# jirsat/wavenets

Hardware: NVIDIA B200
Metric: audio samples/sec fwd+bwd WaveNet stack (higher is better)
Workload: dtype bf16

## Files before the change

### wavenets_b200/csrc/gemm_tc_stack_bwd.cuh

```cuda
#pragma once
#include "gemm_tc_stack.cuh"

#ifdef TC_TIMELINE
#define SBT_DECL(n) long long sbt[n] = {}; long long sbt_prev = clock64();
#define SBT(i) { const long long sbt_now = clock64(); sbt[i] += sbt_now - sbt_prev; sbt_prev = sbt_now; }
#else
#define SBT_DECL(n)
#define SBT(i)
#endif

struct alignas(128) TcStackBwdLayer {
  CUtensorMap tmDX, tmDS, tmWdg, tmZf, tmZs, tmDZ, tmWb, tmDXp, tmO;
  int shift[TC_MAX_TAPS];
  int has_dx, has_ds, has_res;
  int wait_dx;
  const uint8_t* mask;
  int kind, out_mode, act, kb_tap, in_flag_layer;
  int alias;
};

struct TcStackBwdParams {
  int B, T, tiles_t, num_mtiles, L;
  int nseg;
  int kb_dx, kb_ds;
  unsigned long long pol_dx, pol_ds, pol_w, pol_z, pol_dz_ld, pol_dz_st, pol_o;
  float drop_scale;
  int relaxed_handoff;
  int band, nbands;
};

template <int D_, int R_, bool V2 = false> struct TcStackBwdCfg {
  static constexpr int BM = 128, BK = 64;
  static constexpr int A_BYTES = BM * BK * 2;
  static constexpr int B_BYTES = 128 * BK * 2;
  static constexpr int STAGE_BYTES = A_BYTES + B_BYTES;
  static constexpr int STAGES = V2 ? 5 : 3;
  static constexpr int NSLAB = 2 * D_ / 64;
  static constexpr int NPAIR = D_ / 64;
  static constexpr int DZ_SLOTS = V2 ? 0 : 4;
  static constexpr int DZ_BYTES = DZ_SLOTS * A_BYTES;
  static constexpr int PANEL = 128 * 64;
  static constexpr int IN_SLOTS = 3, OUT_SLOTS = 2;
  static constexpr int TMEM_COLS = 512;
  static constexpr int SMEM_BYTES = STAGES * STAGE_BYTES + DZ_BYTES + IN_SLOTS * 2 * PANEL + OUT_SLOTS * PANEL + 512;
  static_assert(D_ % 128 == 0 && D_ <= 256 && R_ % 64 == 0 && R_ <= 256, "stack backward kernel: D in {128,256}, R <= 256");
  static_assert(SMEM_BYTES <= 232448, "stack backward kernel does not fit shared memory");
};

template <int D_, int R_, bool V2>
__global__ void __launch_bounds__(416, 1)
tc_stack_bwd_kernel(const TcStackBwdLayer* __restrict__ layers, int* __restrict__ flags_dx, int* __restrict__ flags_dz, const TcStackBwdParams p) {
  using Cfg = TcStackBwdCfg<D_, R_, V2>;
  constexpr int STAGES = Cfg::STAGES, NEPI = 8, NPAIR = Cfg::NPAIR;
  constexpr int KB_Z = Cfg::NSLAB;
  extern __shared__ __align__(1024) uint8_t smem_sb[];
  uint8_t* smem = smem_sb;
  if ((smem_u32(smem) & 1023u) != 0u) { if (threadIdx.x == 0) printf("libwavenet_b200: dynamic shared memory is not 1024-byte aligned\n"); __trap(); }
  uint8_t* dzbuf = smem + STAGES * Cfg::STAGE_BYTES;
  uint8_t* in_ring = dzbuf + Cfg::DZ_BYTES;
  uint8_t* out_ring = in_ring + Cfg::IN_SLOTS * 2 * Cfg::PANEL;
  uint64_t* full_bar = (uint64_t*)(out_ring + Cfg::OUT_SLOTS * Cfg::PANEL);
  uint64_t* empty_bar = full_bar + STAGES;
  uint64_t* dg_full = empty_bar + STAGES;
  uint64_t* dg_empty = dg_full + 1;
  uint64_t* out_full = dg_empty + 1;
  uint64_t* out_empty = out_full + 1;
  uint64_t* in_full = out_empty + 1;
  uint64_t* in_empty = in_full + Cfg::IN_SLOTS;
  uint64_t* oslot_empty = in_empty + Cfg::IN_SLOTS;
  uint64_t* slab_done = oslot_empty + Cfg::OUT_SLOTS;
  uint64_t* slab_full = slab_done + 2;
  uint64_t* slab_cons = slab_full + 2;
  uint64_t* slab_free = slab_cons + 2;
  uint64_t* a_done = slab_free + 2;
  uint64_t* a_ready = a_done + STAGES;
  uint64_t* sfree = a_ready + STAGES;
  uint32_t* tmem_ptr = (uint32_t*)(sfree + STAGES);
  auto tile_ksteps = [&](const TcStackBwdLayer& Ly, int& n_dg, int& n_un, int& n_sh) {
    if (Ly.kind) { n_dg = 0; n_un = 0; n_sh = p.nseg * Ly.kb_tap; }
    else { n_dg = (Ly.has_dx ? p.kb_dx : 0) + (Ly.has_ds ? p.kb_ds : 0); n_un = KB_Z; n_sh = (p.nseg - 1) * KB_Z; }
  };
  auto ring_adv = [&](int& rs, uint32_t& rp, int n) { rs += n; while (rs >= STAGES) { rs -= STAGES; rp ^= 1u; } };

  const int warp = threadIdx.x >> 5, lane = threadIdx.x & 31;
  const uint32_t crank = cluster_ctarank();
  const bool leader = crank == 0;
  const int tile_first = (int)blockIdx.x >> 1, tile_stride = (int)gridDim.x >> 1;
  const int pair_row0 = (int)crank * Cfg::BM;
  const int total_tiles = p.L * p.num_mtiles;
  const int n_tiles = tile_first < total_tiles ? (total_tiles - tile_first + tile_stride - 1) / tile_stride : 0;

  auto locate = [&](int j, int& ly, int& mt, int& b, int& tb) {
    const int gt = tile_first + j * tile_stride;
    const int full = (p.nbands - 1) * p.band * p.L;
    int lr, mr;
    if (gt < full) {
      const int k = gt / (p.band * p.L), r = gt - k * (p.band * p.L);
      lr = r / p.band; mr = k * p.band + (r - lr * p.band);
    } else {
      const int wl = p.num_mtiles - (p.nbands - 1) * p.band, r = gt - full;
      lr = r / wl; mr = (p.nbands - 1) * p.band + (r - lr * wl);
    }
    ly = p.L - 1 - lr;
    b = mr / p.tiles_t;
    tb = p.tiles_t - 1 - (mr - b * p.tiles_t);
    mt = b * p.tiles_t + tb;
  };

  if (warp == 1 && lane == 0) {
    for (int i = 0; i < STAGES; ++i) { mbar_init(&full_bar[i], 1); mbar_init(&empty_bar[i], 1); }
    mbar_init(dg_full, 1); mbar_init(dg_empty, NEPI * 2); mbar_init(out_full, 1); mbar_init(out_empty, NEPI * 2);
    for (int i = 0; i < Cfg::IN_SLOTS; ++i) { mbar_init(&in_full[i], 1); mbar_init(&in_empty[i], NEPI); }
    for (int i = 0; i < Cfg::OUT_SLOTS; ++i) mbar_init(&oslot_empty[i], 1);
    for (int i = 0; i < 2; ++i) { mbar_init(&slab_done[i], NEPI); mbar_init(&slab_full[i], 2); mbar_init(&slab_cons[i], 1); mbar_init(&slab_free[i], 1); }
    for (int i = 0; i < STAGES; ++i) { mbar_init(&a_done[i], NEPI); mbar_init(&a_ready[i], 2); mbar_init(&sfree[i], 1); }
    mbar_fence_init();
  }
  if (warp == 2) tmem_alloc_pair<Cfg::TMEM_COLS>(tmem_ptr);
  tc_fence_before();
  __syncthreads();
  cluster_sync_all();
  tc_fence_after();
  const uint32_t tmem_base = *tmem_ptr;
  pdl_launch_dependents();
  pdl_wait();

  auto wait_flag = [&](const int* f, int ly, int mt) {
    const long long spin0 = clock64();
    while (ld_acquire_gpu(f) < 2) {
      __nanosleep(32);
      if (clock64() - spin0 > 6000000000ll) { printf("libwavenet_b200: stack backward waited > 3 s for tile (%d, %d)\n", ly, mt); __trap(); }
    }
  };

  if (warp == 0) {
    if (lane == 0) {
      int stage = 0; uint32_t phase = 0;
      auto next = [&]() { if (++stage == STAGES) { stage = 0; phase ^= 1; } };
      uint32_t un_pend = 0u, un_wpar = 0u, un_npar = 0u;
      auto stage_wait = [&]() {
        mbar_wait(&empty_bar[stage], phase ^ 1);
        if (V2 && ((un_pend >> stage) & 1u)) { mbar_wait(&sfree[stage], (un_wpar >> stage) & 1u); un_pend &= ~(1u << stage); }
      };
      SBT_DECL(4)
      constexpr int WDG_BYTES = (D_ / 2) * 64 * 2, WB_BYTES = (R_ / 2) * 64 * 2;
      for (int j = 0; j < n_tiles; ++j) {
        int ly, mt, b, tb;
        locate(j, ly, mt, b, tb);
        const TcStackBwdLayer& Ly = layers[ly];
        const int t0 = tb * (2 * Cfg::BM) + pair_row0;
        if (Ly.kind) {
          for (int s = 0; s < p.nseg; ++s) {
            const int lo = tb * (2 * Cfg::BM) + Ly.shift[s];
            const int t_lo = lo / (2 * Cfg::BM);
            int t_hi = (lo + 2 * Cfg::BM - 1) / (2 * Cfg::BM);
            if (t_hi > p.tiles_t - 1) t_hi = p.tiles_t - 1;
            SBT(0)
            for (int tt = t_lo; tt <= t_hi; ++tt) wait_flag(flags_dx + (size_t)(ly + 1) * p.num_mtiles + b * p.tiles_t + tt, ly + 1, b * p.tiles_t + tt);
            SBT(1)
          }
          fence_proxy_async_global();
          for (int s = 0; s < p.nseg; ++s)
            for (int kb = 0; kb < Ly.kb_tap; ++kb) {
              stage_wait();
              uint8_t* sa = smem + stage * Cfg::STAGE_BYTES;
              if (leader) mbar_expect_tx(&full_bar[stage], 2 * (Cfg::A_BYTES + WB_BYTES));
              tma_load_3d_pair_h(sa, &Ly.tmDZ, &full_bar[stage], kb * 64, t0 + Ly.shift[s], b, p.pol_dz_ld);
              tma_load_2d_pair_h(sa + Cfg::A_BYTES, &Ly.tmWb, &full_bar[stage], (s * Ly.kb_tap + kb) * 64, (int)crank * (R_ / 2), p.pol_w);
              next();
            }
          continue;
        }
        if (Ly.has_dx) {
          if (Ly.wait_dx) {
            SBT(0)
            wait_flag(flags_dx + (size_t)(ly + 1) * p.num_mtiles + mt, ly + 1, mt);
            fence_proxy_async_global();
            SBT(1)
          }
          for (int kb = 0; kb < p.kb_dx; ++kb) {
            stage_wait();
            uint8_t* sa = smem + stage * Cfg::STAGE_BYTES;
            if (leader) mbar_expect_tx(&full_bar[stage], 2 * (Cfg::A_BYTES + WDG_BYTES));
            tma_load_4d_pair_h(sa, &Ly.tmDX, &full_bar[stage], kb * 64, t0, b, 0, p.pol_dx);
            tma_load_2d_pair_h(sa + Cfg::A_BYTES, &Ly.tmWdg, &full_bar[stage], kb * 64, (int)crank * (D_ / 2), p.pol_w);
            next();
          }
        }
        if (Ly.has_ds) {
          const int k0 = (Ly.has_dx && !Ly.alias) ? p.kb_dx * 64 : 0;
          for (int kb = 0; kb < p.kb_ds; ++kb) {
            stage_wait();
            uint8_t* sa = smem + stage * Cfg::STAGE_BYTES;
            if (leader) mbar_expect_tx(&full_bar[stage], 2 * (Cfg::A_BYTES + WDG_BYTES));
            tma_load_4d_pair_h(sa, &Ly.tmDS, &full_bar[stage], kb * 64, t0, b, 0, p.pol_ds);
            tma_load_2d_pair_h(sa + Cfg::A_BYTES, &Ly.tmWdg, &full_bar[stage], k0 + kb * 64, (int)crank * (D_ / 2), p.pol_w);
            next();
          }
        }
        const int kloc = (p.nseg - 1) * 2 * D_;
        for (int pr = 0; pr < NPAIR; ++pr) {
          for (int hh = 0; hh < 2; ++hh) {
            const int slab = hh == 0 ? pr : NPAIR + pr;
            stage_wait();
            uint8_t* sa = smem + stage * Cfg::STAGE_BYTES;
            if (leader) mbar_expect_tx(&full_bar[stage], 2 * WB_BYTES);
            tma_load_2d_pair_h(sa + Cfg::A_BYTES, &Ly.tmWb, &full_bar[stage], kloc + slab * 64, (int)crank * (R_ / 2), p.pol_w);
            if (V2) {
              un_wpar = (un_wpar & ~(1u << stage)) | (((un_npar >> stage) & 1u) << stage);
              un_npar ^= 1u << stage; un_pend |= 1u << stage;
            }
            next();
          }
        }
        for (int s = 0; s < p.nseg - 1; ++s) {
          const int lo = tb * (2 * Cfg::BM) + Ly.shift[s];
          const int t_lo = lo / (2 * Cfg::BM);
          int t_hi = (lo + 2 * Cfg::BM - 1) / (2 * Cfg::BM);
          if (t_hi > p.tiles_t - 1) t_hi = p.tiles_t - 1;
          SBT(0)
          for (int tt = t_lo; tt <= t_hi; ++tt) wait_flag(flags_dz + (size_t)ly * p.num_mtiles + b * p.tiles_t + tt, ly, b * p.tiles_t + tt);
          fence_proxy_async_global();
          SBT(2)
          for (int kb = 0; kb < KB_Z; ++kb) {
            stage_wait();
            uint8_t* sa = smem + stage * Cfg::STAGE_BYTES;
            if (leader) mbar_expect_tx(&full_bar[stage], 2 * (Cfg::A_BYTES + WB_BYTES));
            tma_load_3d_pair_h(sa, &Ly.tmDZ, &full_bar[stage], kb * 64, t0 + Ly.shift[s], b, p.pol_dz_ld);
            tma_load_2d_pair_h(sa + Cfg::A_BYTES, &Ly.tmWb, &full_bar[stage], s * 2 * D_ + kb * 64, (int)crank * (R_ / 2), p.pol_w);
            next();
          }
        }
      }
      SBT(0)
#ifdef TC_TIMELINE
      if (blockIdx.x == 0 || blockIdx.x == 41)
        printf("SBWD cta %d producer: tiles %d  ring+issue %lld  wait_flag_dx %lld  wait_flag_dz %lld\n", blockIdx.x, n_tiles, sbt[0], sbt[1], sbt[2]);
#endif
    }
  } else if (warp == 1) {
    if (leader) {
      constexpr uint32_t idesc_g = umma_idesc_bf16(256, D_, 0, 0);
      constexpr uint32_t idesc_o = umma_idesc_bf16(256, R_, 0, 0);
      const uint32_t t_dg = tmem_base, t_out = tmem_base + 256u;
      int stage = 0; uint32_t phase = 0;
      uint32_t n_sf[2] = {0u, 0u};
      uint32_t ng = 0u;
      uint32_t ar_par = 0u;
      SBT_DECL(10)
      auto kstep = [&](uint32_t d_tmem, uint32_t idesc, bool a_from_dz, int slot, bool first, uint64_t* extra0, uint64_t* extra1) {
#ifdef TC_TIMELINE
        const long long w0 = clock64();
#endif
        mbar_wait(&full_bar[stage], phase);
#ifdef TC_TIMELINE
        sbt[9] += clock64() - w0;
#endif
        tc_fence_after();
        if (elect_one()) {
          const uint32_t sa = smem_u32(smem + stage * Cfg::STAGE_BYTES);
          const uint32_t a_addr = a_from_dz ? smem_u32(dzbuf) + (uint32_t)slot * (uint32_t)Cfg::A_BYTES : sa;
          const uint64_t adesc = umma_smem_desc(a_addr, 16, 1024);
          const uint64_t bdesc = umma_smem_desc(sa + Cfg::A_BYTES, 16, 1024);
#pragma unroll
          for (int k = 0; k < Cfg::BK / 16; ++k)
            umma_bf16_pair(d_tmem, adesc + (uint64_t)(2 * k), bdesc + (uint64_t)(2 * k), idesc, (first && k == 0) ? 0u : 1u);
          umma_commit_pair(&empty_bar[stage]);
          if (extra0) umma_commit_pair(extra0);
          if (extra1) umma_commit_pair(extra1);
        }
        __syncwarp();
        if (++stage == STAGES) { stage = 0; phase ^= 1; }
      };
      for (int j = 0; j < n_tiles; ++j) {
        int ly, mt, b, tb;
        locate(j, ly, mt, b, tb);
        const TcStackBwdLayer& Ly = layers[ly];
        const uint32_t par = (uint32_t)(j & 1);
        if (Ly.kind) {
          SBT(2)
          mbar_wait(out_empty, par ^ 1);
          SBT(3)
          tc_fence_after();
          const int ks_p = p.nseg * Ly.kb_tap;
          for (int ks = 0; ks < ks_p; ++ks) kstep(t_out, idesc_o, false, 0, ks == 0, ks == ks_p - 1 ? out_full : nullptr, nullptr);
          SBT(7)
          continue;
        }
        const uint32_t gpar = ng & 1u; ++ng;
        SBT(0)
        mbar_wait(dg_empty, gpar ^ 1);
        SBT(1)
        tc_fence_after();
        const int ks_dg = (Ly.has_dx ? p.kb_dx : 0) + (Ly.has_ds ? p.kb_ds : 0);
        for (int ks = 0; ks < ks_dg; ++ks) kstep(t_dg, idesc_g, false, 0, ks == 0, ks == ks_dg - 1 ? dg_full : nullptr, nullptr);
        SBT(2)
        mbar_wait(out_empty, par ^ 1);
        SBT(3)
        tc_fence_after();
        const int ks_sh = (p.nseg - 1) * KB_Z;
        bool first = true;
        if constexpr (V2) {
          for (int q = 0; q < KB_Z; ++q) {
            if ((q & 1) == 0) { mbar_wait(&a_ready[stage], (ar_par >> stage) & 1u); ar_par ^= 1u << stage; }
            SBT(5)
            tc_fence_after();
            const bool last = ks_sh == 0 && q == KB_Z - 1;
            kstep(t_out, idesc_o, false, 0, first, last ? out_full : nullptr, nullptr); first = false;
            SBT(6)
          }
        } else
        for (int pr = 0; pr < NPAIR; ++pr) {
          const int ps = pr & 1;
          mbar_wait(&slab_full[ps], n_sf[ps] & 1u); ++n_sf[ps];
          SBT(5)
          tc_fence_after();
          const bool last = ks_sh == 0 && pr == NPAIR - 1;
          kstep(t_out, idesc_o, true, 2 * ps, first, nullptr, nullptr); first = false;
          kstep(t_out, idesc_o, true, 2 * ps + 1, false, &slab_cons[ps], last ? out_full : nullptr);
          SBT(6)
        }
        for (int ks = 0; ks < ks_sh; ++ks) kstep(t_out, idesc_o, false, 0, false, ks == ks_sh - 1 ? out_full : nullptr, nullptr);
        SBT(7)
      }
#ifdef TC_TIMELINE
      if (lane == 0 && (blockIdx.x == 0 || blockIdx.x == 40))
        printf("SBWD cta %d mma: tiles %d  wait_dg_empty %lld  DG ksteps %lld  wait_out_empty %lld  wait_slab_full %lld  unshifted %lld  shifted %lld  (of the ksteps: wait_full_bar %lld)\n",
               blockIdx.x, n_tiles, sbt[1], sbt[2], sbt[3], sbt[5], sbt[6], sbt[7], sbt[9]);
#endif
    }
  } else if (warp == 2) {
    int oslot = 0;
    uint64_t* pend = nullptr;
    uint64_t* pend2 = nullptr;
    auto committed = [&](uint64_t* rel, uint64_t* rel2 = nullptr) {
      bulk_commit_group();
      if (pend) { bulk_wait_group_read<1>(); mbar_arrive(pend); if (pend2) mbar_arrive(pend2); }
      pend = rel; pend2 = rel2;
    };
    int s_rs = 0; uint32_t s_rp = 0u;
    auto publish = [&](int* flag) {
      bulk_wait_group<0>();
      if (pend) { mbar_arrive(pend); if (pend2) mbar_arrive(pend2); pend = nullptr; pend2 = nullptr; }
      fence_proxy_async_global();
      __threadfence();
      red_release_gpu_add(flag, 1);
    };
    for (int j = 0; j < n_tiles; ++j) {
      int ly, mt, b, tb;
      locate(j, ly, mt, b, tb);
      const TcStackBwdLayer& Ly = layers[ly];
      const int t0 = tb * (2 * Cfg::BM) + pair_row0;
      int n_dg, n_un, n_sh;
      tile_ksteps(Ly, n_dg, n_un, n_sh);
      if (!Ly.kind) {
      int u_rs = s_rs; uint32_t u_rp = s_rp;
      ring_adv(u_rs, u_rp, n_dg);
      for (int pr = 0; pr < NPAIR; ++pr) {
        const int ps = pr & 1;
        if constexpr (V2) {
          named_bar_sync(8 + pr, NEPI * 32 + 32);
          const int sf = u_rs; ring_adv(u_rs, u_rp, 1);
          const int ss = u_rs; ring_adv(u_rs, u_rp, 1);
          if (lane == 0) {
            tma_store_3d_h(smem + sf * Cfg::STAGE_BYTES, &Ly.tmDZ, pr * 64, t0, b, p.pol_dz_st);
            tma_store_3d_h(smem + ss * Cfg::STAGE_BYTES, &Ly.tmDZ, D_ + pr * 64, t0, b, p.pol_dz_st);
            committed(&sfree[sf], &sfree[ss]);
          }
        } else {
        named_bar_sync(8 + ps, NEPI * 32 + 32);
        if (lane == 0) {
          tma_store_3d_h(dzbuf + (2 * ps) * Cfg::A_BYTES, &Ly.tmDZ, pr * 64, t0, b, p.pol_dz_st);
          tma_store_3d_h(dzbuf + (2 * ps + 1) * Cfg::A_BYTES, &Ly.tmDZ, D_ + pr * 64, t0, b, p.pol_dz_st);
          committed(&slab_free[ps]);
        }
        }
        __syncwarp();
      }
      if (lane == 0) publish(flags_dz + (size_t)ly * p.num_mtiles + mt);
      __syncwarp();
      }
      for (int step = 0; step < R_ / 32; ++step) {
        named_bar_sync(3 + oslot, NEPI * 32 + 32);
        if (lane == 0) {
          tma_store_3d_h(out_ring + oslot * Cfg::PANEL, &Ly.tmO, step * 32, t0, b, p.pol_o);
          committed(&oslot_empty[oslot]);
        }
        __syncwarp();
        if (++oslot == Cfg::OUT_SLOTS) oslot = 0;
      }
      if (lane == 0) publish(flags_dx + (size_t)ly * p.num_mtiles + mt);
      __syncwarp();
      ring_adv(s_rs, s_rp, n_dg + n_un + n_sh);
    }
    if (lane == 0) bulk_wait_group<0>();
  } else if (warp == 3) {
    if (lane == 0) {
      int islot = 0; uint32_t iphase = 0;
      for (int j = 0; j < n_tiles; ++j) {
        int ly, mt, b, tb;
        locate(j, ly, mt, b, tb);
        const TcStackBwdLayer& Ly = layers[ly];
        const int t0 = tb * (2 * Cfg::BM) + pair_row0;
        if (!Ly.kind)
        for (int step = 0; step < D_ / 32; ++step) {
          mbar_wait(&in_empty[islot], iphase ^ 1);
          mbar_expect_tx(&in_full[islot], 2u * Cfg::PANEL);
          uint8_t* dst = in_ring + islot * 2 * Cfg::PANEL;
          tma_load_3d_h(dst, &Ly.tmZf, &in_full[islot], step * 32, t0, b, p.pol_z);
          tma_load_3d_h(dst + Cfg::PANEL, &Ly.tmZs, &in_full[islot], step * 32, t0, b, p.pol_z);
          if (++islot == Cfg::IN_SLOTS) { islot = 0; iphase ^= 1; }
        }
        if (Ly.out_mode) {
          if (Ly.in_flag_layer >= 0) {
            wait_flag(flags_dx + (size_t)Ly.in_flag_layer * p.num_mtiles + mt, Ly.in_flag_layer, mt);
            fence_proxy_async_global();
          }
          for (int step = 0; step < R_ / 32; ++step) {
            mbar_wait(&in_empty[islot], iphase ^ 1);
            mbar_expect_tx(&in_full[islot], (uint32_t)Cfg::PANEL);
            tma_load_3d_h(in_ring + islot * 2 * Cfg::PANEL, &Ly.tmDXp, &in_full[islot], step * 32, t0, b, p.pol_dx);
            if (++islot == Cfg::IN_SLOTS) { islot = 0; iphase ^= 1; }
          }
        }
      }
    }
  } else if (warp == 12) {
    if (lane == 0) {
      uint32_t n_sd[2] = {0u, 0u};
      int h_rs = 0; uint32_t h_rp = 0u, ad_par = 0u;
      for (int j = 0; j < n_tiles; ++j) {
        int n_dg, n_un, n_sh;
        { int ly, mt, b, tb; locate(j, ly, mt, b, tb); tile_ksteps(layers[ly], n_dg, n_un, n_sh); }
        if constexpr (V2) {
          int u_rs = h_rs; uint32_t u_rp = h_rp;
          ring_adv(u_rs, u_rp, n_dg);
          for (int q = 0; q < n_un; q += 2) {
            mbar_wait(&a_done[u_rs], (ad_par >> u_rs) & 1u); ad_par ^= 1u << u_rs;
            if (leader) mbar_arrive(&a_ready[u_rs]);
            else if (p.relaxed_handoff) mbar_arrive_remote_relaxed(&a_ready[u_rs], 0u);
            else mbar_arrive_remote(&a_ready[u_rs], 0u);
            ring_adv(u_rs, u_rp, 2);
          }
          ring_adv(h_rs, h_rp, n_dg + n_un + n_sh);
          continue;
        }
        if (n_un == 0) continue;
        for (int pr = 0; pr < NPAIR; ++pr) {
          const int ps = pr & 1;
          mbar_wait(&slab_done[ps], n_sd[ps] & 1u); ++n_sd[ps];
          if (leader) mbar_arrive(&slab_full[ps]);
          else if (p.relaxed_handoff) mbar_arrive_remote_relaxed(&slab_full[ps], 0u);
          else mbar_arrive_remote(&slab_full[ps], 0u);
        }
      }
    }
  } else if (warp >= 4 && warp < 12) {
    const int e = warp - 4;
    const int quarter = warp & 3;
    const int q = e >> 2;
    const int row = quarter * 32 + lane;
    const uint32_t row_off = (uint32_t)row * 64u;
    const uint32_t sw = (uint32_t)((row >> 1) & 3);
    const uint32_t u0 = (uint32_t)(2 * q), u1 = u0 + 1;
    const uint32_t off0 = row_off + ((u0 ^ sw) << 4), off1 = row_off + ((u1 ^ sw) << 4);
    const uint32_t grow = (uint32_t)row * 128u, gsw = (uint32_t)(row & 7);
    int islot = 0; uint32_t iphase = 0;
    int oslot = 0; uint32_t ophase = 0;
    uint32_t n_use[2] = {0u, 0u};
    uint32_t nge = 0u;
    int e_rs = 0; uint32_t e_rp = 0u;
    uint32_t eu_pend = 0u, eu_wpar = 0u, eu_npar = 0u;
    uint8_t* slab_dst[2] = {nullptr, nullptr};
    int slab_st[2] = {0, 0};
    const TcEpiGateBwd<true>::Params pg{D_};
    const uint32_t lane_base = (uint32_t)(quarter * 32) << 16;
    SBT_DECL(10)
    for (int j = 0; j < n_tiles; ++j) {
      const uint32_t par = (uint32_t)(j & 1);
      int out_mode, out_act, kind;
      int n_dg, n_un, n_sh;
      const uint8_t* mrow = nullptr;
      {
        int ly, mt, b, tb;
        locate(j, ly, mt, b, tb);
        out_mode = layers[ly].out_mode; out_act = layers[ly].act; kind = layers[ly].kind;
        tile_ksteps(layers[ly], n_dg, n_un, n_sh);
        const int tt = tb * (2 * Cfg::BM) + pair_row0 + row;
        if (layers[ly].mask && tt < p.T && b < p.B) mrow = layers[ly].mask + ((size_t)b * p.T + tt) * R_;
      }
      if (!kind) {
      const uint32_t gpar = nge & 1u; ++nge;
      SBT(0)
      mbar_wait(dg_full, gpar);
      SBT(1)
      tc_fence_after();
      int u_rs = e_rs; uint32_t u_rp = e_rp;
      ring_adv(u_rs, u_rp, n_dg);
      {
        TmemAccRow acc{tmem_base + lane_base, true};
#pragma unroll 1
        for (int step = 0; step < D_ / 32; ++step) {
          const int pr = step >> 1, ps = pr & 1;
          float in[2][16];
          float out[2][16];
          SBT(2)
          mbar_wait(&in_full[islot], iphase);
          SBT(3)
          {
            const uint8_t* ib = in_ring + islot * 2 * Cfg::PANEL;
#pragma unroll
            for (int k = 0; k < 2; ++k) {
              const uint4 a = *reinterpret_cast<const uint4*>(ib + k * Cfg::PANEL + off0);
              const uint4 c = *reinterpret_cast<const uint4*>(ib + k * Cfg::PANEL + off1);
              const uint32_t w[8] = {a.x, a.y, a.z, a.w, c.x, c.y, c.z, c.w};
#pragma unroll
              for (int i = 0; i < 8; ++i) {
                in[k][2 * i] = __uint_as_float(w[i] << 16);
                in[k][2 * i + 1] = __uint_as_float(w[i] & 0xffff0000u);
              }
            }
          }
          __syncwarp();
          if (lane == 0) mbar_arrive(&in_empty[islot]);
          if (++islot == Cfg::IN_SLOTS) { islot = 0; iphase ^= 1; }
          TcEpiGateBwd<true>::chunk(pg, acc, 0, step * 32 + q * 16, 0, 0, 3u, in, out, nullptr);
          SBT(2)
          if constexpr (V2) {
            if ((step & 1) == 0) {
#pragma unroll
              for (int k = 0; k < 2; ++k) {
                mbar_wait(&empty_bar[u_rs], u_rp ^ 1u);
                if ((eu_pend >> u_rs) & 1u) { mbar_wait(&sfree[u_rs], (eu_wpar >> u_rs) & 1u); eu_pend &= ~(1u << u_rs); }
                eu_wpar = (eu_wpar & ~(1u << u_rs)) | (((eu_npar >> u_rs) & 1u) << u_rs);
                eu_npar ^= 1u << u_rs; eu_pend |= 1u << u_rs;
                slab_st[k] = u_rs; slab_dst[k] = smem + u_rs * Cfg::STAGE_BYTES;
                ring_adv(u_rs, u_rp, 1);
              }
            }
          } else
          if ((step & 1) == 0 && n_use[ps] > 0) {
            mbar_wait(&slab_cons[ps], (n_use[ps] - 1u) & 1u);
            mbar_wait(&slab_free[ps], (n_use[ps] - 1u) & 1u);
          }
          SBT(4)
          {
            const int ch = (step & 1) * 32 + q * 16;
            const uint32_t j0 = (uint32_t)(ch >> 3);
#pragma unroll
            for (int k = 0; k < 2; ++k) {
              uint8_t* gs = (V2 ? slab_dst[k] : dzbuf + (2 * ps + k) * Cfg::A_BYTES) + grow;
              uint4 a, c;
              a.x = pack_bf16x2(out[k][0], out[k][1]); a.y = pack_bf16x2(out[k][2], out[k][3]);
              a.z = pack_bf16x2(out[k][4], out[k][5]); a.w = pack_bf16x2(out[k][6], out[k][7]);
              c.x = pack_bf16x2(out[k][8], out[k][9]); c.y = pack_bf16x2(out[k][10], out[k][11]);
              c.z = pack_bf16x2(out[k][12], out[k][13]); c.w = pack_bf16x2(out[k][14], out[k][15]);
              *reinterpret_cast<uint4*>(gs + ((j0 ^ gsw) << 4)) = a;
              *reinterpret_cast<uint4*>(gs + (((j0 + 1) ^ gsw) << 4)) = c;
            }
          }
          if (step & 1) {
            fence_proxy_async();
            named_bar_arrive(8 + (V2 ? pr : ps), NEPI * 32 + 32);
            __syncwarp();
            if constexpr (V2) {
              if (lane == 0) mbar_arrive(&a_done[slab_st[0]]);
            } else {
              if (lane == 0) mbar_arrive(&slab_done[ps]);
            }
            ++n_use[ps];
          }
        }
      }
      tc_fence_before();
      __syncwarp();
      if (lane == 0) mbar_arrive_remote_relaxed(dg_empty, 0u);
      }
      SBT(2)
      mbar_wait(out_full, par);
      SBT(5)
      tc_fence_after();
      {
        TmemAccRow acc{tmem_base + 256u + lane_base, true};
#pragma unroll 1
        for (int step = 0; step < R_ / 32; ++step) {
          float v[16];
          acc.load16(step * 32 + q * 16, v);
          if (mrow) {
            const uint4 mk = __ldg(reinterpret_cast<const uint4*>(mrow + step * 32 + q * 16));
            const uint32_t mw[4] = {mk.x, mk.y, mk.z, mk.w};
#pragma unroll
            for (int i = 0; i < 16; ++i) v[i] = ((mw[i >> 2] >> (8 * (i & 3))) & 0xffu) ? v[i] * p.drop_scale : 0.f;
          }
          if (out_mode) {
            mbar_wait(&in_full[islot], iphase);
            const uint8_t* ib = in_ring + islot * 2 * Cfg::PANEL;
            const uint4 a = *reinterpret_cast<const uint4*>(ib + off0);
            const uint4 c = *reinterpret_cast<const uint4*>(ib + off1);
            const uint32_t w[8] = {a.x, a.y, a.z, a.w, c.x, c.y, c.z, c.w};
            float y[16];
#pragma unroll
            for (int i = 0; i < 8; ++i) {
              y[2 * i] = __uint_as_float(w[i] << 16);
              y[2 * i + 1] = __uint_as_float(w[i] & 0xffff0000u);
            }
            if (out_mode == 1) {
#pragma unroll
              for (int i = 0; i < 16; ++i) v[i] += y[i];
            } else {
              wn_act_grad16(out_act, y, v);
            }
            __syncwarp();
            if (lane == 0) mbar_arrive(&in_empty[islot]);
            if (++islot == Cfg::IN_SLOTS) { islot = 0; iphase ^= 1; }
          }
          uint8_t* ob = out_ring + oslot * Cfg::PANEL;
          SBT(6)
          mbar_wait(&oslot_empty[oslot], ophase ^ 1);
          SBT(7)
          uint4 a, c;
          a.x = pack_bf16x2(v[0], v[1]); a.y = pack_bf16x2(v[2], v[3]); a.z = pack_bf16x2(v[4], v[5]); a.w = pack_bf16x2(v[6], v[7]);
          c.x = pack_bf16x2(v[8], v[9]); c.y = pack_bf16x2(v[10], v[11]); c.z = pack_bf16x2(v[12], v[13]); c.w = pack_bf16x2(v[14], v[15]);
          *reinterpret_cast<uint4*>(ob + off0) = a;
          *reinterpret_cast<uint4*>(ob + off1) = c;
          fence_proxy_async();
          named_bar_arrive(3 + oslot, NEPI * 32 + 32);
          if (++oslot == Cfg::OUT_SLOTS) { oslot = 0; ophase ^= 1; }
        }
      }
      tc_fence_before();
      __syncwarp();
      if (lane == 0) mbar_arrive_remote_relaxed(out_empty, 0u);
      ring_adv(e_rs, e_rp, n_dg + n_un + n_sh);
      SBT(6)
    }
#ifdef TC_TIMELINE
    if (lane == 0 && warp == 4 && (blockIdx.x == 0 || blockIdx.x == 41))
      printf("SBWD cta %d epilogue warp 4: wait_dg_full %lld  DG epi work %lld (+ wait z panels %lld, wait slab slot %lld)  wait_out_full %lld  OUT epi work %lld (+ wait out slot %lld)\n",
             blockIdx.x, sbt[1], sbt[2], sbt[3], sbt[4], sbt[5], sbt[6], sbt[7]);
#endif
  }
  tc_fence_before();
  __syncthreads();
  cluster_sync_all();
  if (warp == 2) tmem_dealloc_pair<Cfg::TMEM_COLS>(tmem_base);
}

struct TcStackBwdDesc {
  int B, T, nseg, shift[TC_MAX_TAPS], D, R, S;
  const bf16* dxo;
  const bf16* dskip; int lds;
  const bf16* z;
  bf16* dz;
  bf16* dx;
  const bf16* Wdg; int k_dg;
  const bf16* Wb; int k_b;
  int has_res;
  const uint8_t* mask; float drop_scale;
  int plain; const bf16* gin;
  int out_mode, act, ein_layer; const bf16* ein;
  int alias;
};

struct TcStackBwdPlan {
  int B = 0, T = 0, L = 0, num_mtiles = 0; bool drop = false;
  TcStackBwdLayer* d_layers = nullptr; int* d_flags = nullptr;
  void release() { cudaFree(d_layers); cudaFree(d_flags); d_layers = nullptr; d_flags = nullptr; }
};

template <int D_, int R_>
static int tc_stack_bwd_build_t(TmapCache& tc, const std::vector<TcStackBwdDesc>& descs, TcStackBwdPlan* plan) {
  std::vector<TcStackBwdLayer> tab(descs.size());
  for (size_t l = 0; l < descs.size(); ++l) {
    const TcStackBwdDesc& d = descs[l];
    TcStackBwdLayer& t = tab[l];
    memset(&t, 0, sizeof(t));
    const TcEpiIo xo{d.dx, d.R, d.R, 0};
    const CUtensorMap* mO = tc_panel_map(tc, xo, d.T, d.B);
    uint64_t bd[2] = {(uint64_t)d.k_b, (uint64_t)d.R}, bs[1] = {(uint64_t)d.k_b * 2};
    uint32_t bb[2] = {64, (uint32_t)(R_ / 2)};
    const CUtensorMap* mWb = tc.get(d.Wb, 2, bd, bs, bb);
    if (!mO || !mWb) return -10;
    t.tmO = *mO; t.tmWb = *mWb; t.tmDXp = *mO;
    for (int s = 0; s < TC_MAX_TAPS; ++s) t.shift[s] = s < d.nseg ? d.shift[s] : 0;
    t.mask = d.mask;
    t.kind = d.plain ? 1 : 0; t.out_mode = d.out_mode; t.act = d.act; t.in_flag_layer = d.out_mode == 1 ? d.ein_layer : -1;
    if (d.out_mode) {
      const TcEpiIo ei{d.ein, d.R, d.R, 0};
      const CUtensorMap* mp = tc_panel_map(tc, ei, d.T, d.B);
      if (!mp) return -10;
      t.tmDXp = *mp;
    }
    if (d.plain) {
      const CUtensorMap* mG = tc_slab_map(tc, d.gin, d.D, d.D, d.T, d.B);
      if (!mG) return -10;
      t.tmDZ = *mG; t.kb_tap = d.D / 64;
      t.tmDX = *mG; t.tmDS = *mG; t.tmWdg = *mWb; t.tmZf = *mO; t.tmZs = *mO;
      continue;
    }
    const CUtensorMap* mDZ = tc_slab_map(tc, d.dz, 2 * d.D, 2 * d.D, d.T, d.B);
    const TcEpiIo zf{d.z, 2 * d.D, d.D, 0}, zs{d.z + d.D, 2 * d.D, d.D, 0};
    const CUtensorMap* mZf = tc_panel_map(tc, zf, d.T, d.B);
    const CUtensorMap* mZs = tc_panel_map(tc, zs, d.T, d.B);
    uint64_t wd[2] = {(uint64_t)d.k_dg, (uint64_t)d.D}, ws[1] = {(uint64_t)d.k_dg * 2};
    uint32_t wb[2] = {64, (uint32_t)(D_ / 2)};
    const CUtensorMap* mWdg = tc.get(d.Wdg, 2, wd, ws, wb);
    if (!mDZ || !mZf || !mZs || !mWdg) return -10;
    t.tmDZ = *mDZ; t.tmZf = *mZf; t.tmZs = *mZs; t.tmWdg = *mWdg;
    t.tmDX = *mDZ; t.tmDS = *mDZ;
    if (d.dxo) {
      const CUtensorMap* m = tc_act_map(tc, d.dxo, d.R, d.R, d.T, d.B, 1, 0, 128);
      if (!m) return -10;
      t.tmDX = *m;
    }
    if (d.dskip) {
      const CUtensorMap* m = tc_act_map(tc, d.dskip, d.lds, d.S, d.T, d.B, 1, 0, 128);
      if (!m) return -10;
      t.tmDS = *m;
    }
    t.has_dx = d.dxo != nullptr; t.has_ds = d.dskip != nullptr; t.has_res = d.out_mode == 1 ? 1 : 0; t.alias = d.alias;
    t.wait_dx = (d.dxo != nullptr && l + 1 < descs.size()) ? 1 : 0;
  }
  const TcStackBwdDesc& d0 = descs[0];
  plan->release();
  plan->B = d0.B; plan->T = d0.T; plan->L = (int)descs.size(); plan->num_mtiles = d0.B * ((d0.T + 255) / 256); plan->drop = false;
  for (const TcStackBwdDesc& d : descs) if (d.mask) plan->drop = true;
  if (cudaMalloc((void**)&plan->d_layers, tab.size() * sizeof(TcStackBwdLayer)) != cudaSuccess ||
      cudaMemcpy(plan->d_layers, tab.data(), tab.size() * sizeof(TcStackBwdLayer), cudaMemcpyHostToDevice) != cudaSuccess ||
      cudaMalloc((void**)&plan->d_flags, (size_t)2 * plan->L * plan->num_mtiles * sizeof(int)) != cudaSuccess) {
    snprintf(g_tc_err, sizeof(g_tc_err), "stack backward: plan allocation failed: %s", cudaGetErrorString(cudaGetLastError()));
    plan->release();
    return -23;
  }
  return 0;
}

template <int D_, int R_, bool V2>
static int tc_stack_bwd_launch_t(cudaStream_t st, const TcStackBwdPlan& plan, const TcStackBwdDesc& d0) {
  using Cfg = TcStackBwdCfg<D_, R_, V2>;
  TcStackBwdParams p{};
  p.B = d0.B; p.T = d0.T; p.tiles_t = (d0.T + 255) / 256; p.num_mtiles = d0.B * p.tiles_t; p.L = plan.L;
  p.nseg = d0.nseg; p.kb_dx = d0.R / 64; p.kb_ds = d0.S / 64; p.drop_scale = d0.drop_scale;
  p.pol_dx = tc_policy(TC_L2_NORMAL); p.pol_ds = tc_policy(TC_L2_LAST); p.pol_w = tc_policy(TC_L2_LAST); p.pol_z = tc_policy(TC_L2_FIRST);
  p.pol_dz_ld = tc_policy(TC_L2_NORMAL); p.pol_dz_st = tc_policy(TC_L2_LAST); p.pol_o = tc_policy(TC_L2_LAST);
  auto kern = tc_stack_bwd_kernel<D_, R_, V2>;
  static unsigned long long attr_devs = 0ull;
  if (tc_first_use_on_device(&attr_devs)) {
    cudaError_t e = cudaFuncSetAttribute(kern, cudaFuncAttributeMaxDynamicSharedMemorySize, Cfg::SMEM_BYTES);
    if (e != cudaSuccess) { snprintf(g_tc_err, sizeof(g_tc_err), "cudaFuncSetAttribute(smem=%d): %s", Cfg::SMEM_BYTES, cudaGetErrorString(e)); return -12; }
  }
  const int pairs = tc_num_sms() / 2;
  if (p.num_mtiles <= pairs) return -100;
  {
    static int relaxed = -1;
    if (relaxed < 0) { const char* e = getenv("WN_TC_HANDOFF_RELAXED"); relaxed = (e && e[0] == '1') ? 1 : 0; }
    p.relaxed_handoff = relaxed;
    static int band_target = -1;
    if (band_target < 0) { const char* e = getenv("WN_TC_SB_BAND"); band_target = e ? atoi(e) : 128; }
    int nb = band_target > 0 ? p.num_mtiles / band_target : 1;
    if (nb < 1) nb = 1;
    for (; nb > 1; --nb) {
      const int bw = (p.num_mtiles + nb - 1) / nb;
      if (bw > pairs && p.num_mtiles - (nb - 1) * bw > pairs) break;
    }
    p.nbands = nb; p.band = (p.num_mtiles + nb - 1) / nb;
  }
  {
    static int max_clusters_dev[64];
    static unsigned long long mc_devs = 0ull;
    int& max_clusters = max_clusters_dev[tc_current_device()];
    if (tc_first_use_on_device(&mc_devs)) {
      cudaLaunchConfig_t oc{};
      oc.gridDim = dim3(tc_num_sms()); oc.blockDim = dim3(416); oc.dynamicSmemBytes = Cfg::SMEM_BYTES;
      cudaLaunchAttribute oa[1];
      oa[0].id = cudaLaunchAttributeClusterDimension;
      oa[0].val.clusterDim.x = 2; oa[0].val.clusterDim.y = 1; oa[0].val.clusterDim.z = 1;
      oc.attrs = oa; oc.numAttrs = 1;
      int n = 0;
      if (cudaOccupancyMaxActiveClusters(&n, kern, &oc) != cudaSuccess) { n = 0; cudaGetLastError(); }
      max_clusters = n;
    }
    if (pairs > max_clusters) return -100;
  }
  const size_t nflags = (size_t)plan.L * plan.num_mtiles;
  if (cudaMemsetAsync(plan.d_flags, 0, 2 * nflags * sizeof(int), st) != cudaSuccess) return -14;
  cudaLaunchConfig_t cfg{};
  cfg.gridDim = dim3(2 * pairs); cfg.blockDim = dim3(416); cfg.dynamicSmemBytes = Cfg::SMEM_BYTES; cfg.stream = st;
  cudaLaunchAttribute attr[2];
  cfg.attrs = attr; cfg.numAttrs = tc_launch_attrs(attr, 2);
  cudaError_t e = cudaLaunchKernelEx(&cfg, kern, (const TcStackBwdLayer*)plan.d_layers, plan.d_flags, plan.d_flags + nflags, p);
  if (e != cudaSuccess) { snprintf(g_tc_err, sizeof(g_tc_err), "stack backward launch: %s", cudaGetErrorString(e)); return -13; }
  return 0;
}

static inline int tc_stack_bwd_build(TmapCache& tc, const std::vector<TcStackBwdDesc>& descs, TcStackBwdPlan* plan) {
  const TcStackBwdDesc& d = descs[0];
  if (d.D == 256 && d.R == 256) return tc_stack_bwd_build_t<256, 256>(tc, descs, plan);
  if (d.D == 128 && d.R == 128) return tc_stack_bwd_build_t<128, 128>(tc, descs, plan);
  return -100;
}
static inline int tc_stack_bwd_launch(cudaStream_t st, const TcStackBwdPlan& plan, const TcStackBwdDesc& d, bool v2) {
  if (d.D == 256 && d.R == 256) return v2 ? tc_stack_bwd_launch_t<256, 256, true>(st, plan, d) : tc_stack_bwd_launch_t<256, 256, false>(st, plan, d);
  if (d.D == 128 && d.R == 128) return v2 ? tc_stack_bwd_launch_t<128, 128, true>(st, plan, d) : tc_stack_bwd_launch_t<128, 128, false>(st, plan, d);
  return -100;
}
```

### wavenets_b200/csrc/wn_api.cu

```cuda
#include <cuda_runtime.h>
#include <math.h>
#include <stdarg.h>
#include <stdio.h>
#include <stdlib.h>
#include <string.h>

#include <algorithm>
#include <string>
#include <vector>

#include "../../include/wavenet_b200.h"
#include "common.cuh"
#include "epilogues.cuh"
#include "gemm_simt.cuh"
#include "gemm_tc.cuh"
#include "gemm_tc_block.cuh"
#include "gemm_tc_wgroup.cuh"
#include "gemm_tc_stack.cuh"
#include "gemm_tc_stack_bwd.cuh"
#include "kernels_misc.cuh"
#include "generate.cuh"
#include "nccl_dl.cuh"

static thread_local char g_err[512] = "";
static void set_err(const char* fmt, ...) {
  va_list ap;
  va_start(ap, fmt);
  vsnprintf(g_err, sizeof(g_err), fmt, ap);
  va_end(ap);
}
extern "C" const char* wn_last_error(void) { return g_err; }
extern "C" const char* wn_build_info(void) {
  return "libwavenet_b200 sm_100a; fp32 FFMA tier + bf16 tcgen05/TMEM/TMA tier; built " __DATE__ " " __TIME__;
}

#define CK(expr)                                                                          \
  do {                                                                                    \
    cudaError_t e_ = (expr);                                                              \
    if (e_ != cudaSuccess) {                                                              \
      set_err("CUDA error %s (%s) at %s:%d", cudaGetErrorName(e_), cudaGetErrorString(e_), __FILE__, __LINE__); \
      return WN_ERR_CUDA;                                                                 \
    }                                                                                     \
  } while (0)
#define RET(expr)              \
  do {                         \
    int r_ = (expr);           \
    if (r_ != WN_OK) return r_; \
  } while (0)

static inline int cdiv(long long a, long long b) { return (int)((a + b - 1) / b); }
static inline int rup(int a, int b) { return (a + b - 1) / b * b; }

struct ParamInfo {
  std::string name;
  int shape[3];
  int ndim;
  long long offset, count;
};

struct ConvP {
  int K = 1, cin = 0, cout = 0, dil = 1;
  int w_idx = -1, b_idx = -1;
  bool gate = false;
  float* Wf = nullptr; int Npad = 0;
  float* Wb = nullptr; int Cpad = 0;
  bf16* Wf16 = nullptr; int Kf16 = 0;
  bf16* Wb16 = nullptr; int Kb16 = 0;
  int N16 = 0, C16 = 0, tileN16 = 0;
};

struct BlockP {
  std::vector<ConvP> stack;
  ConvP conv1;
  bool has_skip = false;
  ConvP conv_skip;
  bool has_cond = false;
  int cw_idx = -1, cb_idx = -1;
  float* Wdg = nullptr; int Dpad = 0;
  bf16* Wdg16 = nullptr;
  bf16* Wres16 = nullptr;
  float* Wfc = nullptr;
  float* Wct = nullptr; int Ccpad = 0;
  bf16* Wfc16 = nullptr; int Kfc16 = 0;
  bf16* Wct16 = nullptr; int Cc16 = 0, tileCc16 = 0;
};

struct Arena {
  char* base = nullptr;
  size_t cap = 0, off = 0;
  bool dry = true;
  void* take(size_t bytes) {
    off = (off + 255) & ~(size_t)255;
    void* p = dry ? nullptr : base + off;
    off += bytes;
    return p;
  }
};

struct wn_handle {
  wn_config cfg;
  int R, D, S, Sp , K, L, Cc, Cout;
  bool alias_skip;
  std::vector<int> dil;
  int rf;
  std::vector<ParamInfo> params;
  long long n_scalars = 0;
  float* d_params = nullptr;
  float* d_grads = nullptr;
  ConvP input_conv;
  std::vector<BlockP> blocks;
  std::vector<ConvP> head;
  std::vector<int> map_w, map_b, map_width;
  float* Wskip = nullptr; int Spad = 0;
  bf16* Wskip16 = nullptr;
  float* bskip_sum = nullptr;
  int* d_bskip_offsets = nullptr;
  int* d_cond_offsets = nullptr;
  Arena pack, ws;
  int maxB, maxT;
  void* h0 = nullptr;
  std::vector<std::vector<void*>> acts;
  std::vector<void*> zbuf, xout;
  void* G_all = nullptr;
  void* skipsum = nullptr;
  std::vector<void*> hact;
  float* logits = nullptr; int ldl = 0;
  void* dlogits = nullptr; int ldd = 0;
  void *dhA = nullptr, *dhB = nullptr;
  void* dskip = nullptr;
  void *dxA = nullptr, *dxB = nullptr, *dotmp = nullptr;
  void *dcatA = nullptr, *dcatB = nullptr;
  void* dz = nullptr;
  void *dpA = nullptr, *dpB = nullptr;
  float* colpart = nullptr; int col_chunks = 0;
  float* wg_partial = nullptr; long long wg_partial_elems = 0;
  float* cs_partial = nullptr;
  float* wg_partial_side = nullptr; float* cs_partial_side = nullptr;
  void* dz2 = nullptr;
  float* loss_partial = nullptr; int loss_parts_cap = 0;
  float* cond_act[WN_MAX_LIST + 1] = {};
  float* cond_dact = nullptr;
  float* cond_dact2 = nullptr;
  float* cb = nullptr;
  float* dcb = nullptr;
  float* dcond = nullptr;
  float* l2_sum = nullptr;
  uint8_t* drop_mask = nullptr;
  std::vector<void*> xdrop;
  void* ddrop = nullptr;
  unsigned long long* d_drop_ctr = nullptr;
  unsigned long long drop_seed = 0x243F6A8885A308D3ull;
  bool drop_injected = false;
  bool drop_active = false;
  float* opt_m = nullptr; float* opt_v = nullptr;
  OptChunk* opt_chunks = nullptr; int opt_n_chunks = 0;
  int* opt_var_first = nullptr;
  float* opt_partial = nullptr; float* opt_scale = nullptr; float* opt_norms = nullptr;
  float opt_lr = 1e-3f, opt_b1 = 0.9f, opt_b2 = 0.999f, opt_eps = 1e-7f, opt_clipnorm = 0.f;
  long long opt_t = 0;
  float* layer_xin = nullptr;
  void* layer_in = nullptr;
  float* d_loss = nullptr;
  float* d_frames = nullptr; float* d_cond_in = nullptr;
  float* pin_frames = nullptr; float* pin_cond = nullptr; float* pin_loss = nullptr;
  cudaStream_t own_stream = nullptr;
  int lastB = 0, lastT = 0;
  bool fwd_valid = false;
  bool layer_fwd_valid[WN_MAX_DILATIONS] = {};
  bool layer_drop[WN_MAX_DILATIONS] = {};
  int Ccs = 0;
  std::vector<void*> cseq;
  float* cseq_bias = nullptr;
  float* cseq_dw = nullptr;
  const void* layer_cseq[WN_MAX_DILATIONS] = {};
  const void* cond_seq = nullptr;
  const float* last_cond = nullptr;
  long long launches = 0;
  int prof_tag = 0;
  std::vector<std::pair<cudaEvent_t, cudaEvent_t>> prof_events;
  std::vector<const char*> prof_labels;
  const char* cur_label = "misc";
  const char* outer_label = nullptr;
  std::vector<float> prof_ms;
  std::vector<const char*> prof_last_labels;
  size_t prof_used = 0;
  long long prof_launches = 0;
  TmapCache tmaps;
  struct StepGraph { const float* frames; const float* cond; int B, T, nrep; float* loss; bool train; int seen; long long launches; cudaGraphExec_t exec; };
  std::vector<StepGraph> graphs;
  int use_graphs = 1;
  cudaEvent_t ev_in = nullptr, ev_out = nullptr;
  cudaStream_t side_stream = nullptr;
  std::vector<cudaEvent_t> ev_blk_in, ev_blk_dz, ev_blk_done;
  int use_side = 1;
  int use_res_gemm = 1;
  int use_fused_fwd = 1;
  int stack_fwd_layers = 0;
  int use_stack_fwd = 1;
  std::vector<TcStackPlan> stack_plans;
  int use_stack_bwd = 2, stack_bwd_layers = 0;
  std::vector<TcStackBwdPlan> stack_bwd_plans;
  int tile_gate_bwd = 0, tile_dgrad = 0;
  int fused_fwd_launches = 0;
  int use_group_wgrad = 0;
  void* dz_all = nullptr;
  void* dx_all = nullptr;
  void* do_all = nullptr;
  std::vector<std::vector<void*>> dp_keep;
  struct WgPlan { int B, T; bool drop; bool sb; int nb; TcWgGroupPlan plan; };
  std::vector<WgPlan> wg_plans;
  std::vector<TcWgJobDesc> wg_jobs;
  int dskip_l2_last = 0;
  int wg_last_tiles = 0, wg_last_side = 0;
  int wg_last_partials = 0;
  int wg_cur_group = -1;
  int wg_side_every = 5;
  cudaEvent_t ev_wg_side = nullptr;
  int wg_force_split = 0, wg_pair_tiles = 1;
  int use_merged_finish = 0;
  struct Gen {
    int B = 0, cap = 0;
    float* audio = nullptr; std::vector<std::vector<float*>> hist; float* z = nullptr; float* skipsum = nullptr;
    std::vector<float*> hbuf; float* logits = nullptr; float* sampled = nullptr; int* t_dev = nullptr;
    std::vector<float*> wcat, bcat;
    std::vector<void*> allocs;
  } gen;
  TcWgradFinish pend_finish{}; bool pend_valid = false; int pend_blocks = 0; long long pend_partial_elems = 0, pend_cs_elems = 0;
  std::vector<PackJob> pack_jobs;
  PackJob* d_pack_jobs = nullptr; long long pack_blocks = 0; bool pack_ready = false;
  wn_ncclComm_t comm = nullptr; bool comm_owned = false; int comm_nranks = 1, comm_rank = 0;
  int ar_in_step = 0;
  int ar_buckets = 2;
  int ar_first_pct = 70;
  bool ar_now = false;
  long long ar_early_lo = -1, ar_early_hi = -1;
  cudaStream_t comm_stream = nullptr;
  cudaEvent_t ev_bucket[8] = {nullptr, nullptr, nullptr, nullptr, nullptr, nullptr, nullptr, nullptr};
  cudaEvent_t ev_comm_done = nullptr;
  int wg_cur_bucket = 0;
  int last_ar_buckets = 0;
  bool cond_wgrad_done = false;
};

enum { CLS_DILATED = 1, CLS_GEMM = 2, CLS_LOSS = 3, CLS_MISC = 4 };

struct LaunchScope {
  wn_handle* h; cudaStream_t st; bool timed = false; size_t slot = 0;
  LaunchScope(wn_handle* h_, cudaStream_t st_, int cls) : h(h_), st(st_) {
    h->launches++;
    const int t = h->prof_tag;
    if (t && ((t == 1 && cls == CLS_DILATED) || (t == 2 && (cls == CLS_DILATED || cls == CLS_GEMM)) || (t == 3 && cls == CLS_LOSS) ||
              (t == 4))) {
      if (h->prof_used == h->prof_events.size()) {
        cudaEvent_t a, b;
        cudaEventCreate(&a); cudaEventCreate(&b);
        h->prof_events.push_back({a, b});
      }
      slot = h->prof_used++;
      if (h->prof_labels.size() <= slot) h->prof_labels.resize(slot + 1);
      h->prof_labels[slot] = h->outer_label ? h->outer_label : h->cur_label;
      cudaEventRecord(h->prof_events[slot].first, st);
      timed = true;
      h->prof_launches++;
    }
  }
  ~LaunchScope() {
    if (timed) cudaEventRecord(h->prof_events[slot].second, st);
  }
};

struct OuterLabel {
  wn_handle* h; const char* prev;
  OuterLabel(wn_handle* h_, const char* l) : h(h_), prev(h_->outer_label) { h->outer_label = l; }
  ~OuterLabel() { h->outer_label = prev; }
};

static int add_param(wn_handle* h, const std::string& name, std::initializer_list<int> shape) {
  ParamInfo p;
  p.name = name;
  p.ndim = (int)shape.size();
  p.count = 1;
  int i = 0;
  for (int s : shape) { p.shape[i++] = s; p.count *= s; }
  for (; i < 3; ++i) p.shape[i] = 1;
  p.offset = h->n_scalars;
  h->n_scalars += (p.count + 3) / 4 * 4;
  h->params.push_back(p);
  return (int)h->params.size() - 1;
}

static int validate_config(const wn_config& c) {
  if (c.conditioning != 0 && c.conditioning != 1) { set_err("Conditioning must be 'global', 'local' or None."); return c.conditioning == 2 ? WN_ERR_UNSUPPORTED : WN_ERR_VALUE; }
  if (c.kernel_size < 2) { set_err("Kernel size must be at least 2."); return WN_ERR_VALUE; }
  if (c.dilation_bound < 1) { set_err("dilation bound must be power of kernel_size."); return WN_ERR_VALUE; }
  {
    long long v = 1; bool ok = false;
    for (int i = 0; i < 40 && v <= c.dilation_bound; ++i) { if (v == c.dilation_bound) { ok = true; break; } v *= c.kernel_size; }
    if (!ok && c.n_dilations == 0) { set_err("dilation bound must be power of kernel_size."); return WN_ERR_VALUE; }
  }
  if (c.layers_per_block < 1) { set_err("Layers per block must be at least 1."); return WN_ERR_VALUE; }
  if (c.blocks < 1) { set_err("Blocks must be at least 1."); return WN_ERR_VALUE; }
  if (c.num_mixtures < 0) { set_err("Number of mixtures must be at least 1 or None."); return WN_ERR_VALUE; }
  if (c.dropout < 0 || c.dropout > 1) { set_err("Dropout must be between 0 and 1."); return WN_ERR_VALUE; }
  if (c.sampling_function < 0 || c.sampling_function > 2) { set_err("Sampling function must be categorical, logistic or gaussian."); return WN_ERR_VALUE; }
  if (c.sampling_function == WN_CATEGORICAL && c.num_mixtures != 0) { set_err("Categorical sampling cannot be used with mixtures."); return WN_ERR_VALUE; }
  if (c.has_head && c.sampling_function != WN_CATEGORICAL && c.num_mixtures == 0) { set_err("mixture sampling needs num_mixtures"); return WN_ERR_VALUE; }
  if (c.channels < 1 || c.max_batch < 1 || c.max_time < 1) { set_err("channels / max_batch / max_time must be positive"); return WN_ERR_VALUE; }
  if (c.kernel_size > WN_MAX_TAPS) { set_err("kernel_size > %d not built", WN_MAX_TAPS); return WN_ERR_UNSUPPORTED; }
  if (c.num_mixtures > WN_MAX_MIX) { set_err("num_mixtures > %d not built", WN_MAX_MIX); return WN_ERR_UNSUPPORTED; }
  if (c.blocks * c.layers_per_block > WN_MAX_DILATIONS) { set_err("too many dilated convs"); return WN_ERR_UNSUPPORTED; }
  if (c.n_mapping < 0 || c.n_mapping > WN_MAX_LIST || c.n_final < 0 || c.n_final > WN_MAX_LIST) { set_err("list too long"); return WN_ERR_VALUE; }
  if (c.has_head && c.sampling_function == WN_CATEGORICAL && (c.bits < 1 || c.bits > 16)) { set_err("bits must be in 1..16"); return WN_ERR_VALUE; }
  if (c.conditioning && c.cond_in < 1) { set_err("conditioning needs cond_in >= 1"); return WN_ERR_VALUE; }
  if (c.precision != WN_FP32 && c.precision != WN_BF16) { set_err("unknown precision"); return WN_ERR_VALUE; }
  return WN_OK;
}

static ConvP make_conv(wn_handle* h, const std::string& pfx, int K, int cin, int cout, int dil, bool gate) {
  ConvP c;
  c.K = K; c.cin = cin; c.cout = cout; c.dil = dil; c.gate = gate;
  c.w_idx = add_param(h, pfx + "/kernel", {K, cin, cout});
  c.b_idx = add_param(h, pfx + "/bias", {cout});
  return c;
}

template <class T> static size_t esz() { return sizeof(T); }

static void layout_buffers(wn_handle* h) {
  const bool bf = h->cfg.precision == WN_BF16;
  const size_t es = bf ? 2 : 4;
  Arena& P = h->pack;
  auto lay_conv = [&](ConvP& c) {
    if (!bf) {
      c.Npad = rup(c.cout, 64);
      c.Wf = (float*)P.take((size_t)c.K * c.cin * c.Npad * 4);
      c.Cpad = rup(c.cin, 64);
      c.Wb = (float*)P.take((size_t)c.K * c.cout * c.Cpad * 4);
    } else {
      tc_pick_tile(c.cout, c.gate, &c.N16, &c.tileN16);
      c.Kf16 = c.K * c.cin;
      c.Wf16 = (bf16*)P.take((size_t)c.N16 * c.Kf16 * 2);
      int tn;
      tc_pick_tile(c.cin, false, &c.C16, &tn);
      c.Kb16 = c.K * c.cout;
      c.Wb16 = (bf16*)P.take((size_t)c.C16 * rup(c.Kb16, 64) * 2);
    }
  };
  if (h->cfg.has_input_conv) {  }
  for (auto& b : h->blocks) {
    for (auto& c : b.stack) lay_conv(c);
    lay_conv(b.conv1);
    if (b.has_skip) lay_conv(b.conv_skip);
    const int rs = h->R + (b.has_skip ? h->S : 0);
    if (!bf) {
      b.Dpad = rup(h->D, 64);
      b.Wdg = (float*)P.take((size_t)rs * b.Dpad * 4);
    } else {
      int n16, tn;
      tc_pick_tile(h->D, false, &n16, &tn);
      b.Dpad = n16;
      b.Wdg16 = (bf16*)P.take((size_t)n16 * rup(rs, 64) * 2);
      if (h->cfg.use_residual) b.Wres16 = (bf16*)P.take((size_t)b.conv1.N16 * (h->D + h->R) * 2);
    }
    if (b.has_cond && h->Ccs > 0) {
      const ConvP& c = b.stack.back();
      if (!bf) {
        b.Wfc = (float*)P.take((size_t)(c.K * c.cin + h->Cc) * c.Npad * 4);
        b.Ccpad = rup(h->Cc, 64);
        b.Wct = (float*)P.take((size_t)c.cout * b.Ccpad * 4);
      } else {
        b.Kfc16 = c.K * c.cin + h->Ccs;
        b.Wfc16 = (bf16*)P.take((size_t)c.N16 * b.Kfc16 * 2);
        tc_pick_tile(h->Cc, false, &b.Cc16, &b.tileCc16);
        b.Wct16 = (bf16*)P.take((size_t)b.Cc16 * c.cout * 2);
      }
    }
  }
  for (auto& c : h->head) lay_conv(c);
  if (!bf) {
    h->Spad = rup(h->Sp, 64);
    h->Wskip = (float*)P.take((size_t)h->L * h->D * h->Spad * 4);
  } else {
    int tn;
    tc_pick_tile(h->Sp, false, &h->Spad, &tn);
    h->Wskip16 = (bf16*)P.take((size_t)h->Spad * h->L * h->D * 2);
  }
  h->bskip_sum = (float*)P.take((size_t)h->Sp * 4);
  h->d_bskip_offsets = (int*)P.take((size_t)h->L * 4 * 2);
  h->d_cond_offsets = (int*)P.take((size_t)h->L * 4 * 2);

  Arena& W = h->ws;
  const size_t rows = (size_t)h->maxB * h->maxT;
  const int R = h->R, D = h->D, Sp = h->Sp, L = h->L;
  h->h0 = W.take(rows * R * es);
  h->acts.assign(L, {});
  h->zbuf.assign(L, nullptr);
  h->xout.assign(L, nullptr);
  for (int l = 0; l < L; ++l) {
    const int depth = (int)h->blocks[l].stack.size();
    h->acts[l].assign(depth - 1 > 0 ? depth - 1 : 0, nullptr);
    for (int j = 0; j + 1 < depth; ++j) h->acts[l][j] = W.take(rows * D * es);
    h->zbuf[l] = W.take(rows * 2 * D * es);
    h->xout[l] = W.take(rows * R * es);
  }
  h->G_all = W.take((size_t)L * rows * D * es);
  h->skipsum = W.take(rows * Sp * es);
  int maxhead = Sp > R ? Sp : R;
  h->hact.assign(h->head.size() > 0 ? h->head.size() - 1 : 0, nullptr);
  for (size_t i = 0; i + 1 < h->head.size(); ++i) {
    h->hact[i] = W.take(rows * h->head[i].cout * es);
    if (h->head[i].cout > maxhead) maxhead = h->head[i].cout;
  }
  if (h->cfg.has_head) {
    h->ldl = h->Cout;
    h->logits = (float*)W.take(rows * h->ldl * 4);
    h->ldd = bf ? rup(h->Cout, 64) : h->Cout;
    h->dlogits = W.take(rows * h->ldd * es);
    h->dhA = W.take(rows * maxhead * es);
    h->dhB = W.take(rows * maxhead * es);
  }
  h->dskip = W.take(rows * Sp * es);
  h->dxA = W.take(rows * R * es);
  h->dxB = W.take(rows * R * es);
  h->dotmp = W.take(rows * R * es);
  if (h->use_group_wgrad) {
    h->dz_all = W.take((size_t)L * rows * 2 * D * es);
    h->dx_all = W.take((size_t)L * rows * R * es);
    if (h->alias_skip && h->cfg.use_skip) h->do_all = W.take((size_t)L * rows * R * es);
    h->dp_keep.assign(L, {});
    for (int l = 0; l < L; ++l) {
      const int depth = (int)h->blocks[l].stack.size();
      for (int j = 0; j + 1 < depth; ++j) h->dp_keep[l].push_back(W.take(rows * D * es));
    }
  } else if (bf && !h->alias_skip && h->cfg.use_skip) {
    h->dcatA = W.take(rows * (size_t)(R + h->S) * es);
    h->dcatB = W.take(rows * (size_t)(R + h->S) * es);
  }
  h->dz = W.take(rows * 2 * D * es);
  h->dz2 = W.take(rows * 2 * D * es);
  h->dpA = W.take(rows * D * es);
  h->dpB = W.take(rows * D * es);
  h->col_chunks = cdiv(h->maxT, 64);
  int nmax = 2 * D;
  if (R > nmax) nmax = R;
  if (Sp > nmax) nmax = Sp;
  for (auto& c : h->head) if (c.cout > nmax) nmax = c.cout;
  const int kin = (h->K + 1);
  size_t colpart_elems = (size_t)h->maxB * h->col_chunks * (nmax > kin * R ? nmax : kin * R);
  h->colpart = (float*)W.take(colpart_elems * 4);
  long long maxkn = 0;
  auto upd = [&](long long k, long long n) { if ((k + 1) * n > maxkn) maxkn = (k + 1) * n; };
  for (auto& b : h->blocks) {
    for (auto& c : b.stack) upd((long long)c.K * c.cin, c.cout);
    upd(D, R);
    if (b.has_skip) upd(D, h->S);
    if (b.has_cond && h->Ccs > 0) upd(h->Ccs, 2 * D);
  }
  for (auto& c : h->head) upd(c.cin, c.cout);
  h->wg_partial_elems = maxkn * WN_MAX_WGRAD_SPLITS;
  h->wg_partial = (float*)W.take((size_t)h->wg_partial_elems * 4 * 2);
  h->wg_partial_side = (float*)W.take((size_t)h->wg_partial_elems * 4 * 2);
  if (bf) {
    int max_mt = 1;
    auto mt = [&](int K, int cin) { const int m = K * cdiv(cin, 128); if (m > max_mt) max_mt = m; };
    for (auto& b : h->blocks) { for (auto& c : b.stack) mt(c.K, c.cin); mt(1, D); }
    if (h->Ccs > 0) mt(1, h->Ccs);
    for (auto& c : h->head) mt(1, c.cin);
    h->cs_partial = (float*)W.take((size_t)tc_wgrad_cs_rows(h->maxB, h->maxT, max_mt) * (size_t)rup(nmax, 4) * 4 * 2);
    h->cs_partial_side = (float*)W.take((size_t)tc_wgrad_cs_rows(h->maxB, h->maxT, max_mt) * (size_t)rup(nmax, 4) * 4 * 2);
  }
  h->loss_parts_cap = cdiv((long long)rows, 8) + 8;
  h->loss_partial = (float*)W.take((size_t)h->loss_parts_cap * 4);
  int maxw = h->cfg.cond_in;
  for (int i = 0; i < h->cfg.n_mapping; ++i) if (h->cfg.mapping_layers[i] > maxw) maxw = h->cfg.mapping_layers[i];
  if (h->cfg.conditioning) {
    for (int i = 0; i < h->cfg.n_mapping; ++i) h->cond_act[i] = (float*)W.take((size_t)h->maxB * h->cfg.mapping_layers[i] * 4);
    h->cond_dact = (float*)W.take((size_t)h->maxB * maxw * 4);
    h->cond_dact2 = (float*)W.take((size_t)h->maxB * maxw * 4);
    h->cb = (float*)W.take((size_t)L * h->maxB * 2 * D * 4);
    h->dcb = (float*)W.take((size_t)L * h->maxB * 2 * D * 4);
    h->dcond = (float*)W.take((size_t)h->maxB * (h->Cc > 0 ? h->Cc : 1) * 4);
  }
  if (h->Ccs > 0) {
    h->cseq.assign(L, nullptr);
    if (bf) {
      for (int l = 0; l < L; ++l) h->cseq[l] = W.take(rows * h->Ccs * 2);
      h->cseq_dw = (float*)W.take((size_t)h->Ccs * 2 * D * 4);
    }
    h->cseq_bias = (float*)W.take((size_t)L * 2 * D * 4);
  }
  h->l2_sum = (float*)W.take(16);
  if (h->cfg.dropout > 0.f) {
    h->drop_mask = (uint8_t*)W.take((size_t)L * rows * R);
    h->xdrop.assign(L, nullptr);
    for (int l = 0; l < L; ++l) h->xdrop[l] = W.take(rows * R * es);
    h->ddrop = W.take(rows * R * es);
    h->d_drop_ctr = (unsigned long long*)W.take(16);
  }
  h->d_loss = (float*)W.take(16);
  h->layer_in = W.take(rows * R * es);
  h->d_frames = (float*)W.take((size_t)h->maxB * (h->maxT + 1) * 4);
  h->d_cond_in = (float*)W.take((size_t)h->maxB * (h->cfg.cond_in > 0 ? h->cfg.cond_in : 1) * 4);
}
// ... 1088 lines not shown
      for (int k = 0; k < c.K; ++k) g.seg[k] = SegH{dcur, dcw, +(c.K - 1 - k) * c.dil, c.cout};
      fill_w(g, c, true);
      g.tile16 = h->tile_dgrad;
      typename EpiActBwd<T, T>::Params ep{};
      ep.N = c.cin;
      if (j > 0) {
        void* dst = group ? h->dp_keep[l][j - 1] : ((dcur == h->dpA) ? h->dpB : h->dpA);
        ep.out = (T*)dst; ep.ldo = D; ep.add = nullptr; ep.y = (const T*)h->acts[l][j - 1]; ep.ldy = D; ep.act = h->cfg.activation;
        ep.vec = vec_ok<T>(D);
        g.l2_in[1] = TC_L2_FIRST; g.l2_out[0] = TC_L2_LAST;
        RET((run_conv_gemm<T, EpiActBwd<T, T>>(h, st, CLS_DILATED, g, ep)));
        dcur = dst;
        dcw = D;
      } else if (h->drop_active) {
        ep.out = (T*)h->ddrop; ep.ldo = R; ep.add = nullptr; ep.y = nullptr; ep.act = ACT_LINEAR; ep.vec = vec_ok<T>(R);
        RET((run_conv_gemm<T, EpiActBwd<T, T>>(h, st, CLS_DILATED, g, ep)));
        if (sd && sd->wait_dx) CK(cudaStreamWaitEvent(st, sd->wait_dx, 0));
        LaunchScope ls(h, st, CLS_MISC);
        dropout_bwd<T><<<cdiv(nR, 256), 256, 0, st>>>((const T*)h->ddrop, h->drop_mask + (size_t)l * rows_cap * R,
                                                     (h->cfg.use_residual && dxout) ? (const T*)dxout : nullptr, ldxo, (T*)dx_in, ldxi,
                                                     (long long)B * Tn, R, 1.0f / (1.0f - h->cfg.dropout));
      } else {
        ep.out = (T*)dx_in; ep.ldo = ldxi;
        ep.add = (h->cfg.use_residual && dxout) ? (const T*)dxout : nullptr; ep.lda = ldxo;
        ep.y = nullptr; ep.act = ACT_LINEAR; ep.vec = vec_ok<T>(R);
        g.l2_in[0] = TC_L2_FIRST; g.l2_out[0] = TC_L2_LAST;
        if (sd && sd->wait_dx) CK(cudaStreamWaitEvent(st, sd->wait_dx, 0));
        RET((run_conv_gemm<T, EpiActBwd<T, T>>(h, st, CLS_DILATED, g, ep)));
      }
    }
  }
  if (h->pend_valid) {
    LaunchScope ls(h, s1, CLS_GEMM);
    tc_wgrad_finish<<<h->pend_blocks, 256, 0, s1>>>(h->pend_finish);
    h->pend_valid = false;
  }
  if (sd) CK(cudaEventRecord(sd->ev_done, sd->side));
  return WN_OK;
}

static int cond_backward(wn_handle* h, cudaStream_t st, const float* cond_in, const float* cond, int B, int l0, int nl, bool run_mapping, float* dcond_out,
                         float l2coef, bool skip_wgrad = false) {
  const int n = 2 * h->D;
  if (l0 == 0 && nl == h->L) {
    if (!skip_wgrad) {
      LaunchScope ls(h, st, CLS_MISC);
      cond_wgrad_all<<<dim3(cdiv((h->Cc + 1) * n, 128), h->L), 128, 0, st>>>(cond, h->Cc, h->dcb, (long long)h->maxB * n, h->d_params, h->d_grads,
                                                                          h->d_cond_offsets, B, n, l2coef, 0);
    }
    {
      LaunchScope ls(h, st, CLS_MISC);
      cond_dgrad_all<<<B * h->Cc, 256, 0, st>>>(h->dcb, (long long)h->maxB * n, h->d_params, h->d_cond_offsets, dcond_out, h->L, B, h->Cc, n);
    }
  } else
  for (int l = l0; l < l0 + nl; ++l) {
    const BlockP& b = h->blocks[l];
    const float* d = h->dcb + (size_t)l * h->maxB * n;
    {
      LaunchScope ls(h, st, CLS_MISC);
      dense_small_wgrad<<<cdiv((h->Cc + 1) * n, 128), 128, 0, st>>>(cond, h->Cc, d, n, G_(h, b.cw_idx), G_(h, b.cb_idx), B, h->Cc, n);
    }
    if (l2coef != 0.f) {
      LaunchScope ls(h, st, CLS_MISC);
      const long long cnt = h->params[b.cw_idx].count;
      reduce_parts<<<cdiv(cnt, 256), 256, 0, st>>>(G_(h, b.cw_idx), 1, 0, G_(h, b.cw_idx), cnt, P_(h, b.cw_idx), l2coef);
    }
    {
      LaunchScope ls(h, st, CLS_MISC);
      dense_small_dgrad<<<cdiv(B * h->Cc, 4), 128, 0, st>>>(d, n, P_(h, b.cw_idx), dcond_out, h->Cc, B, h->Cc, n, l != l0);
    }
  }
  if (!run_mapping) return WN_OK;
  MapArgs ma;
  if (dcond_out == h->dcond && mapping_args(h, cond_in, B, l2coef, &ma)) {
    LaunchScope ls(h, st, CLS_MISC);
    mapping_bwd_fused<<<1, 256, 0, st>>>(ma);
    return WN_OK;
  }
  float* dcur = dcond_out;
  for (int i = (int)h->map_w.size() - 1; i >= 0; --i) {
    const int nn = h->map_width[i];
    const int kin = i > 0 ? h->map_width[i - 1] : h->cfg.cond_in;
    const float* inp = i > 0 ? h->cond_act[i - 1] : cond_in;
    {
      LaunchScope ls(h, st, CLS_MISC);
      dense_small_actgrad<<<cdiv(B * nn, 128), 128, 0, st>>>(dcur, h->cond_act[i], B * nn, h->cfg.mapping_activation);
    }
    {
      LaunchScope ls(h, st, CLS_MISC);
      dense_small_wgrad<<<cdiv((kin + 1) * nn, 128), 128, 0, st>>>(inp, kin, dcur, nn, G_(h, h->map_w[i]), G_(h, h->map_b[i]), B, kin, nn);
    }
    if (l2coef != 0.f) {
      LaunchScope ls(h, st, CLS_MISC);
      const long long cnt = h->params[h->map_w[i]].count;
      reduce_parts<<<cdiv(cnt, 256), 256, 0, st>>>(G_(h, h->map_w[i]), 1, 0, G_(h, h->map_w[i]), cnt, P_(h, h->map_w[i]), l2coef);
    }
    if (i > 0) {
      float* dn = (dcur == h->cond_dact) ? h->cond_dact2 : h->cond_dact;
      LaunchScope ls(h, st, CLS_MISC);
      dense_small_dgrad<<<cdiv(B * kin, 4), 128, 0, st>>>(dcur, nn, P_(h, h->map_w[i]), dn, kin, B, kin, nn, 0);
      dcur = dn;
    }
  }
  return WN_OK;
}

static const BwdSide* side_setup(wn_handle* h, cudaStream_t st, int l, bool on, BwdSide* sd) {
  if (!on) return nullptr;
  sd->side = h->side_stream;
  sd->ev_in = h->ev_blk_in[l]; sd->ev_dz = h->ev_blk_dz[l]; sd->ev_done = h->ev_blk_done[l];
  sd->wait_dz = l + 2 < h->L ? h->ev_blk_done[l + 2] : nullptr;
  sd->wait_dx = l + 1 < h->L ? h->ev_blk_done[l + 1] : nullptr;
  cudaEventRecord(sd->ev_in, st);
  return sd;
}

template <class T>
static int model_backward(wn_handle* h, cudaStream_t st, const float* x, int ldx, const float* cond_in, int B, int Tn, float l2coef) {
  const wn_config& c = h->cfg;
  const bool group = sizeof(T) == 2 && h->use_group_wgrad;
  const bool use_side = sizeof(T) == 2 && h->use_side && h->prof_tag == 0 && h->side_stream != nullptr && !group;
  const bool cat = sizeof(T) == 2 && h->dcatA != nullptr;
  const int ldc = h->R + h->S;
  const size_t rows_cap = (size_t)h->maxB * h->maxT;
  auto dz_of = [&](int l) -> void* { return (T*)h->dz_all + (size_t)l * rows_cap * 2 * h->D; };
  auto dx_of = [&](int l) -> void* { return (T*)h->dx_all + (size_t)l * rows_cap * h->R; };
  h->wg_jobs.clear();
  h->wg_last_tiles = 0; h->wg_last_side = 0;
  bool sb_ok = false;
  if constexpr (sizeof(T) == 2) {
    sb_ok = group && !cat && h->use_stack_bwd && tc_cta_group() == 2 && h->L >= 2 && h->D == h->R && (h->D == 256 || h->D == 128) &&
            h->K <= TC_MAX_TAPS && B * cdiv(Tn, 256) > tc_num_sms() / 2;
    for (auto& b : h->blocks) {
      if (!sb_ok) break;
      sb_ok = b.stack[0].cin % 64 == 0 && (!b.has_skip || h->S % 64 == 0) && b.stack.size() <= 16 &&
              (b.stack.size() == 1 || (h->D == 256 && h->dp_keep.size() == (size_t)h->L));
      for (size_t j = 0; sb_ok && j + 1 < b.stack.size(); ++j) sb_ok = b.stack[j].cout == h->D && b.stack[j].Wb16 != nullptr && b.stack[j].K == h->K;
    }
  }
  h->stack_bwd_layers = 0;
  int side_pairs = 0;
  if (group && !sb_ok && h->use_side && h->side_stream != nullptr && h->wg_side_every > 0) {
    const int pairs = tc_num_sms() / 2, tiles = B * cdiv(Tn, 256);
    if (tiles > pairs) {
      const int rounds = cdiv(tiles, pairs);
      side_pairs = pairs - cdiv(tiles, rounds);
    }
    if (side_pairs < 6) side_pairs = 0;
  }
  auto side_group_of = [&](int l) -> int { return (side_pairs > 0 && (h->L - 1 - l) % h->wg_side_every == 0) ? (h->L - 1 - l) / h->wg_side_every : -1; };
  const int nb = (group && sb_ok && h->ar_now && h->prof_tag == 0 && h->comm_stream != nullptr) ? std::min(std::min(h->ar_buckets, h->L), 8) : 1;
  auto bucket_of = [&](int l) -> int {
    if (nb <= 1) return 0;
    if (nb == 2) return (h->L - 1 - l) * 100 < h->L * h->ar_first_pct ? 0 : 1;
    return ((h->L - 1 - l) * nb) / h->L;
  };
  auto block_off = [&](int l) -> long long {
    if (l < h->L) return h->params[h->blocks[l].stack[0].w_idx].offset;
    if (!h->head.empty()) return h->params[h->head[0].w_idx].offset;
    if (!h->map_w.empty()) return h->params[h->map_w[0]].offset;
    return h->n_scalars;
  };
  h->ar_early_lo = h->ar_early_hi = -1;
  h->last_ar_buckets = 0;
  TcWgGroupPlan* wplan = nullptr;
  if (group) for (auto& wp : h->wg_plans) if (wp.B == B && wp.T == Tn && wp.drop == h->drop_active && wp.sb == sb_ok && wp.nb == nb) wplan = &wp.plan;
  const bool side_now = wplan != nullptr && side_pairs > 0 && h->prof_tag == 0 && !wplan->side.empty();
  g_tc_balance = side_now ? 1 : 0;
  const void* dcur = h->dlogits;
  int dw = h->ldd;
  for (int i = (int)h->head.size() - 1; i >= 0; --i) {
    OuterLabel ol_head(h, "head_bwd");
    const ConvP& hc = h->head[i];
    const void* a_in;
    int a_w;
    if (i > 0) { a_in = h->hact[i - 1]; a_w = h->head[i - 1].cout; }
    else if (c.use_skip) { a_in = h->skipsum; a_w = h->Sp; }
    else { a_in = h->xout[h->L - 1]; a_w = h->R; }
    bool head_grouped = false;
    if constexpr (sizeof(T) == 2) {
      if (group && h->head.size() <= 3 && tc_wgrad_group_ok(hc.cin, hc.cout) && a_w == hc.cin) {
        TcWgJobDesc j{};
        j.A = (const bf16*)a_in; j.lda = a_w; j.cin = hc.cin; j.ntaps = 1; j.shift[0] = 0;
        j.G = (const bf16*)dcur; j.ldg = dw; j.N = hc.cout;
        j.dst = G_(h, hc.w_idx); j.w = c.l2_reg_factor > 0.f ? P_(h, hc.w_idx) : nullptr; j.bias = G_(h, hc.b_idx);
        j.group = -1; j.bucket = nb - 1;
        h->wg_jobs.push_back(j);
        head_grouped = true;
      }
    }
    if (!head_grouped) {
      WgradH w{};
      w.bias_dst = G_(h, hc.b_idx);
      w.B = B; w.T = Tn; w.N = hc.cout; w.G = dcur; w.ldg = dw; w.nseg = 1; w.seg[0] = SegH{a_in, a_w, 0, hc.cin};
      w.dst = G_(h, hc.w_idx); w.w = P_(h, hc.w_idx); w.l2coef = l2coef;
      RET(run_wgrad<T>(h, st, CLS_GEMM, w));
    }
    GemmH g;
    g.B = B; g.T = Tn; g.N = hc.cin; g.nseg = 1;
    g.seg[0] = SegH{dcur, dw, 0, (sizeof(T) == 2 && i + 1 == (int)h->head.size()) ? h->ldd : hc.cout};
    fill_w(g, hc, true);
    typename EpiActBwd<T, T>::Params ep{};
    ep.N = hc.cin; ep.add = nullptr;
    void* dst;
    if (i > 0) {
      dst = (dcur == h->dhA) ? h->dhB : h->dhA;
      ep.out = (T*)dst; ep.ldo = hc.cin; ep.y = (const T*)h->hact[i - 1]; ep.ldy = hc.cin; ep.act = c.activation; ep.vec = vec_ok<T>(hc.cin);
    } else if (cat) {
      dst = (T*)h->dcatA + h->R;
      ep.out = (T*)dst; ep.ldo = ldc; ep.y = nullptr; ep.act = ACT_LINEAR; ep.vec = vec_ok<T>(ldc);
    } else {
      dst = c.use_skip ? h->dskip : (group ? dx_of(h->L - 1) : h->dxA);
      ep.out = (T*)dst; ep.ldo = hc.cin; ep.y = nullptr; ep.act = ACT_LINEAR; ep.vec = vec_ok<T>(hc.cin);
    }
    RET((run_conv_gemm<T, EpiActBwd<T, T>>(h, st, CLS_GEMM, g, ep)));
    dcur = dst;
    dw = hc.cin;
  }
  const void* dxout;
  int ld_dx;
  if (cat) {
    CK(cudaMemcpy2DAsync((T*)h->dcatB + h->R, (size_t)ldc * sizeof(T), (const T*)h->dcatA + h->R, (size_t)ldc * sizeof(T), (size_t)h->S * sizeof(T),
                         (size_t)B * Tn, cudaMemcpyDeviceToDevice, st));
    const void* cur = nullptr;
    void* nxt = h->dcatB;
    for (int l = h->L - 1; l >= 0; --l) {
      const void* x_in = l > 0 ? h->xout[l - 1] : h->h0;
      const void* dsk = cur ? (const void*)((const T*)cur + h->R) : (const void*)((const T*)h->dcatA + h->R);
      BwdSide sd; const BwdSide* sdp = side_setup(h, st, l, use_side, &sd);
      RET(block_backward<T>(h, st, l, x_in, cur, ldc, dsk, ldc, nxt, ldc, B, Tn, l2coef, (l & 1) ? h->dz2 : h->dz, sdp));
      cur = nxt;
      nxt = (nxt == h->dcatB) ? h->dcatA : h->dcatB;
    }
    dxout = cur; ld_dx = ldc;
  } else {
    const void* dskip = c.use_skip ? h->dskip : nullptr;
    dxout = c.use_skip ? nullptr : (group ? dx_of(h->L - 1) : h->dxA);
    bool stacked = false;
    if constexpr (sizeof(T) == 2) {
      if (sb_ok) {
        std::vector<TcStackBwdDesc> bdescs;
        {
          int conv_index = 0;
          for (int l = 0; l < h->L; ++l) {
            BlockP& b = h->blocks[l];
            const int depth = (int)b.stack.size();
            const bf16* blk_dxo = l == h->L - 1 ? (const bf16*)dxout : (const bf16*)dx_of(l);
            bf16* blk_dx = (bf16*)(l > 0 ? dx_of(l - 1) : h->dxA);
            const int next_first = conv_index + depth;
            const bool dxo_in_launch = blk_dxo != nullptr && l < h->L - 1;
            for (int j = 0; j < depth; ++j, ++conv_index) {
              const ConvP& cv = b.stack[j];
              TcStackBwdDesc d{};
              const bool alias = h->alias_skip && dskip != nullptr;
              d.B = B; d.T = Tn; d.nseg = cv.K; d.D = h->D; d.R = h->R; d.S = dskip ? (alias ? h->R : h->S) : 0;
              for (int k = 0; k < cv.K; ++k) d.shift[k] = (cv.K - 1 - k) * cv.dil;
              d.Wb = cv.Wb16; d.k_b = rup(cv.Kb16, 64);
              d.drop_scale = h->drop_active ? 1.0f / (1.0f - c.dropout) : 0.f;
              d.ein_layer = -1;
              d.dx = j == 0 ? blk_dx : (bf16*)h->dp_keep[l][j - 1];
              if (j == 0) {
                if (c.use_residual && blk_dxo) { d.out_mode = 1; d.ein = blk_dxo; d.ein_layer = dxo_in_launch ? next_first : -1; }
                if (h->drop_active) d.mask = h->drop_mask + (size_t)l * rows_cap * h->R;
              } else {
                d.out_mode = 2; d.act = c.activation; d.ein = (const bf16*)h->acts[l][j - 1];
              }
              if (j < depth - 1) {
                d.plain = 1; d.gin = (const bf16*)h->dp_keep[l][j];
              } else {
                d.dxo = blk_dxo;
                d.dskip = ((b.has_skip || alias) && dskip) ? (const bf16*)dskip : nullptr; d.lds = h->Sp;
                d.alias = alias ? 1 : 0;
                d.z = (const bf16*)h->zbuf[l]; d.dz = (bf16*)dz_of(l);
                const int rs = h->R + (b.has_skip ? h->S : 0), koff = (d.dxo || alias) ? 0 : h->R;
                d.Wdg = b.Wdg16 + koff; d.k_dg = rup(rs, 64);
                d.has_res = (c.use_residual && depth == 1) ? 1 : 0;
              }
              bdescs.push_back(d);
            }
          }
        }
        TcStackBwdPlan* sp = nullptr;
        for (auto& q : h->stack_bwd_plans) if (q.B == B && q.T == Tn && q.drop == h->drop_active) sp = &q;
        int r = 0;
        if (!sp) {
          cudaStreamCaptureStatus cs = cudaStreamCaptureStatusNone;
          cudaStreamIsCapturing(st, &cs);
          if (cs == cudaStreamCaptureStatusNone) {
            if (h->stack_bwd_plans.size() >= 4) {
              CK(cudaDeviceSynchronize());
              for (auto& g : h->graphs) if (g.exec) cudaGraphExecDestroy(g.exec);
              h->graphs.clear();
              for (auto& q : h->stack_bwd_plans) q.release();
              h->stack_bwd_plans.clear();
            }
            h->stack_bwd_plans.push_back(TcStackBwdPlan{});
            r = tc_stack_bwd_build(h->tmaps, bdescs, &h->stack_bwd_plans.back());
            if (r == 0) sp = &h->stack_bwd_plans.back(); else h->stack_bwd_plans.pop_back();
          }
        }
        if (sp) {
          struct Label { wn_handle* h; Label(wn_handle* h_) : h(h_) { h->cur_label = "stack_bwd"; } ~Label() { h->cur_label = "misc"; } } lab(h);
          LaunchScope ls(h, st, CLS_DILATED);
          r = tc_stack_bwd_launch(st, *sp, bdescs[0], h->use_stack_bwd >= 2);
          if (r == 0) { stacked = true; h->stack_bwd_layers = h->L; }
          else if (r == -100) h->launches--;
          else { set_err("stack backward launch failed (%d): %s", r, tc_last_error()); return WN_ERR_CUDA; }
        } else if (r != 0 && r != -100) { set_err("stack backward plan failed (%d): %s", r, tc_last_error()); return WN_ERR_CUDA; }
      }
    }
    for (int l = h->L - 1; l >= 0; --l) {
      const void* x_in = l > 0 ? h->xout[l - 1] : h->h0;
      void* dx_in = group ? (l > 0 ? dx_of(l - 1) : h->dxA) : ((dxout == h->dxA) ? h->dxB : h->dxA);
      BwdSide sd; const BwdSide* sdp = side_setup(h, st, l, use_side, &sd);
      h->wg_cur_group = side_group_of(l);
      h->wg_cur_bucket = bucket_of(l);
      RET(block_backward<T>(h, st, l, x_in, dxout, h->R, dskip, h->Sp, dx_in, h->R, B, Tn, l2coef, group ? dz_of(l) : ((l & 1) ? h->dz2 : h->dz), sdp,
                            group, stacked));
      if constexpr (sizeof(T) == 2) {
        if (side_now && h->wg_cur_group >= 0 && h->wg_cur_group < (int)wplan->side.size() && wplan->side[h->wg_cur_group].second > 0) {
          CK(cudaEventRecord(h->ev_blk_dz[l], st));
          CK(cudaStreamWaitEvent(h->side_stream, h->ev_blk_dz[l], 0));
          struct Label { wn_handle* h; Label(wn_handle* h_, const char* lb) : h(h_) { h->cur_label = lb; } ~Label() { h->cur_label = "misc"; } } lab(h, "wgrad_group");
          LaunchScope ls(h, h->side_stream, CLS_DILATED);
          int r = tc_wgrad_group_launch(h->side_stream, *wplan, wplan->side[h->wg_cur_group].first, wplan->side[h->wg_cur_group].second);
          if (r != 0) { set_err("grouped wgrad side launch failed (%d): %s", r, tc_last_error()); return WN_ERR_CUDA; }
          h->wg_last_side++;
        }
      }
      dxout = dx_in;
    }
    h->wg_cur_group = -1; h->wg_cur_bucket = 0;
    ld_dx = h->R;
  }
  g_tc_balance = 0;
  bool input_conv_done = false;
  auto input_conv_bwd = [&](cudaStream_t s_) {
    OuterLabel ol(h, "input_conv_bwd");
    const bool wide = h->R % 2 == 0 && h->R / 2 <= 256 && ld_dx % 2 == 0;
    const int chunks = cdiv(Tn, 64);
    const int nparts = wide ? cdiv((long long)B * Tn, ICB_ROWS) : B * chunks;
    {
      LaunchScope ls(h, s_, CLS_MISC);
      if (wide)
        input_conv_bwd_stage1_wide<T><<<nparts, 256, 0, s_>>>(x, ldx, (const T*)dxout, ld_dx, h->colpart, B, Tn, h->R, h->K);
      else
        input_conv_bwd_stage1<T><<<dim3(cdiv(h->R, 64), chunks, B), 64, 0, s_>>>(x, ldx, (const T*)dxout, ld_dx, h->colpart, B, Tn, h->R, h->K, 64);
    }
    const long long kr = (long long)h->K * h->R;
    {
      LaunchScope ls(h, s_, CLS_MISC);
      reduce_parts_tall<<<cdiv(kr, 32), 256, 0, s_>>>(h->colpart, nparts, (long long)(h->K + 1) * h->R, G_(h, h->input_conv.w_idx), kr,
                                                   l2coef != 0.f ? P_(h, h->input_conv.w_idx) : nullptr, l2coef);
    }
    {
      LaunchScope ls(h, s_, CLS_MISC);
      reduce_parts_tall<<<cdiv(h->R, 32), 256, 0, s_>>>(h->colpart + kr, nparts, (long long)(h->K + 1) * h->R, G_(h, h->input_conv.b_idx), h->R, nullptr, 0.f);
    }
  };
  const bool icb_side = !side_now && h->stack_bwd_layers > 0 && h->use_side && h->side_stream != nullptr && h->prof_tag == 0 && group && !h->wg_jobs.empty();
  if (side_now || icb_side) {
    CK(cudaEventRecord(h->ev_blk_in[0], st));
    CK(cudaStreamWaitEvent(h->side_stream, h->ev_blk_in[0], 0));
    input_conv_bwd(h->side_stream);
    input_conv_done = true;
    if (!(group && !h->wg_jobs.empty())) { CK(cudaEventRecord(h->ev_wg_side, h->side_stream)); CK(cudaStreamWaitEvent(st, h->ev_wg_side, 0)); }
  }
  if constexpr (sizeof(T) == 2) {
    if (group && !h->wg_jobs.empty()) {
      TcWgGroupPlan* plan = wplan;
      if (!plan) {
        cudaStreamCaptureStatus cs = cudaStreamCaptureStatusNone;
        cudaStreamIsCapturing(st, &cs);
        if (cs != cudaStreamCaptureStatusNone) { set_err("grouped wgrad: no plan for (%d, %d) while capturing", B, Tn); return WN_ERR_STATE; }
        if (h->wg_plans.size() >= 4) {
          CK(cudaDeviceSynchronize());
          for (auto& g : h->graphs) if (g.exec) cudaGraphExecDestroy(g.exec);
          h->graphs.clear();
          for (auto& wp : h->wg_plans) wp.plan.release();
          h->wg_plans.clear();
        }
        h->wg_plans.push_back(wn_handle::WgPlan{B, Tn, h->drop_active, sb_ok, nb, TcWgGroupPlan{}});
        plan = &h->wg_plans.back().plan;
        int r = tc_wgrad_group_build(h->tmaps, h->wg_jobs, B, Tn, h->wg_force_split, h->wg_pair_tiles != 0, side_pairs, plan);
        if (r != 0) { h->wg_plans.pop_back(); set_err("grouped wgrad plan failed (%d): %s", r, tc_last_error()); return WN_ERR_CUDA; }
      }
      bool cond_wgrad_done = false;
      if (nb > 1 && (int)plan->buckets.size() == nb && !side_now) {
        struct Label { wn_handle* h; Label(wn_handle* h_, const char* l) : h(h_) { h->cur_label = l; } ~Label() { h->cur_label = "misc"; } } lab(h, "wgrad_group");
        h->wg_last_tiles = plan->ntiles; h->wg_last_partials = plan->npartial;
        for (int k = 0; k < nb; ++k) {
          const TcWgGroupPlan::Bucket& bk = plan->buckets[k];
          {
            LaunchScope ls(h, st, CLS_DILATED);
            int r = tc_wgrad_group_launch(st, *plan, bk.unit0, bk.nunits);
            if (r != 0) { set_err("grouped wgrad launch failed (%d): %s", r, tc_last_error()); return WN_ERR_CUDA; }
          }
          {
            OuterLabel ol(h, "wgrad_group_finish");
            LaunchScope ls(h, st, CLS_DILATED);
            int r = tc_wgrad_group_finish_launch(st, *plan, l2coef, k);
            if (r != 0) { set_err("grouped wgrad finish failed (%d): %s", r, tc_last_error()); return WN_ERR_CUDA; }
          }
          int l_lo = h->L, l_hi = -1;
          for (int l = 0; l < h->L; ++l) if (bucket_of(l) == k) { if (l < l_lo) l_lo = l; if (l > l_hi) l_hi = l; }
          if (c.conditioning && l_hi >= l_lo) {
            OuterLabel ol(h, "cond_bwd");
            LaunchScope ls(h, st, CLS_MISC);
            const int n = 2 * h->D;
            cond_wgrad_all<<<dim3(cdiv((h->Cc + 1) * n, 128), l_hi - l_lo + 1), 128, 0, st>>>(h->last_cond, h->Cc, h->dcb, (long long)h->maxB * n, h->d_params,
                                                                                         h->d_grads, h->d_cond_offsets, B, n, l2coef, l_lo);
          }
          if (k + 1 < nb && l_hi >= l_lo) {
            const long long lo = block_off(l_lo), hi = block_off(l_hi + 1);
            CK(cudaEventRecord(h->ev_bucket[k], st));
            CK(cudaStreamWaitEvent(h->comm_stream, h->ev_bucket[k], 0));
            h->launches++;
            const int r = g_nccl.AllReduce(h->d_grads + lo, h->d_grads + lo, (size_t)(hi - lo), WN_NCCL_FLOAT32, WN_NCCL_SUM, h->comm, h->comm_stream);
            if (r != 0) { set_err("ncclAllReduce (bucket %d) failed (%d): %s", k, r, nccl_errstr(r)); return WN_ERR_CUDA; }
            h->last_ar_buckets++;
            if (h->ar_early_lo < 0 || lo < h->ar_early_lo) h->ar_early_lo = lo;
            if (hi > h->ar_early_hi) h->ar_early_hi = hi;
          }
        }
        cond_wgrad_done = c.conditioning != 0;
      } else
      {
        struct Label { wn_handle* h; Label(wn_handle* h_, const char* l) : h(h_) { h->cur_label = l; } ~Label() { h->cur_label = "misc"; } } lab(h, "wgrad_group");
        {
          LaunchScope ls(h, st, CLS_DILATED);
          h->wg_last_tiles = plan->ntiles; h->wg_last_partials = plan->npartial;
          int r = tc_wgrad_group_launch(st, *plan, 0, side_now ? plan->final_units : plan->nunits);
          if (r != 0) { set_err("grouped wgrad launch failed (%d): %s", r, tc_last_error()); return WN_ERR_CUDA; }
        }
        if (side_now) {
          CK(cudaEventRecord(h->ev_wg_side, h->side_stream));
          CK(cudaStreamWaitEvent(st, h->ev_wg_side, 0));
        }
        {
          OuterLabel ol(h, "wgrad_group_finish");
          LaunchScope ls(h, st, CLS_DILATED);
          int r = tc_wgrad_group_finish_launch(st, *plan, l2coef);
          if (r != 0) { set_err("grouped wgrad finish failed (%d): %s", r, tc_last_error()); return WN_ERR_CUDA; }
        }
      }
      h->cond_wgrad_done = cond_wgrad_done;
    }
  }
  if (icb_side) {
    CK(cudaEventRecord(h->ev_wg_side, h->side_stream));
    CK(cudaStreamWaitEvent(st, h->ev_wg_side, 0));
  }
  if (use_side) CK(cudaStreamWaitEvent(st, h->ev_blk_done[0], 0));
  if (!input_conv_done) input_conv_bwd(st);
  if (c.conditioning) { OuterLabel ol(h, "cond_bwd"); RET(cond_backward(h, st, cond_in, h->last_cond, B, 0, h->L, true, h->dcond, l2coef, h->cond_wgrad_done)); }
  h->cond_wgrad_done = false;
  return WN_OK;
}

static void drop_graphs_fwd(wn_handle* h) {
  cudaDeviceSynchronize();
  for (auto& g : h->graphs) if (g.exec) cudaGraphExecDestroy(g.exec);
  h->graphs.clear();
}

static int check_bt(wn_handle* h, int B, int T) {
  if (!h) { set_err("null handle"); return WN_ERR_VALUE; }
  if (B < 1 || T < 1 || B > h->maxB || T > h->maxT) {
    set_err("batch/time (%d,%d) outside the workspace built for (%d,%d)", B, T, h->maxB, h->maxT);
    return WN_ERR_VALUE;
  }
  return WN_OK;
}

static int gen_alloc(wn_handle* h, int B, int cap) {
  wn_handle::Gen& G = h->gen;
  if (G.B >= B && G.cap >= cap) return WN_OK;
  for (void* a : G.allocs) cudaFree(a);
  G.allocs.clear();
  auto take = [&](size_t bytes) -> void* { void* p = nullptr; if (cudaMalloc(&p, bytes) != cudaSuccess) return nullptr; cudaMemset(p, 0, bytes); G.allocs.push_back(p); return p; };
  G.B = B; G.cap = cap;
  const size_t rows = (size_t)B * cap;
  G.audio = (float*)take(rows * 4);
  G.hist.assign(h->L + 1, {});
  bool ok = G.audio != nullptr;
  for (int l = 0; l <= h->L && ok; ++l) {
    const int depth = l < h->L ? (int)h->blocks[l].stack.size() : 1;
    G.hist[l].assign(depth, nullptr);
    for (int j = 0; j < depth && ok; ++j) { G.hist[l][j] = (float*)take(rows * (j == 0 ? h->R : h->D) * 4); ok = G.hist[l][j] != nullptr; }
  }
  G.z = (float*)take((size_t)B * 2 * h->D * 4);
  G.skipsum = (float*)take((size_t)B * h->Sp * 4);
  G.hbuf.assign(h->head.size(), nullptr);
  for (size_t i = 0; i + 1 < h->head.size() && ok; ++i) { G.hbuf[i] = (float*)take((size_t)B * h->head[i].cout * 4); ok = G.hbuf[i] != nullptr; }
  G.logits = (float*)take((size_t)B * h->Cout * 4);
  G.sampled = (float*)take((size_t)B * 4);
  G.t_dev = (int*)take(16);
  G.wcat.assign(h->L, nullptr); G.bcat.assign(h->L, nullptr);
  for (int l = 0; l < h->L && ok; ++l) {
    if (!(h->cfg.use_skip && h->blocks[l].has_skip)) continue;
    G.wcat[l] = (float*)take((size_t)h->D * (h->R + h->S) * 4);
    G.bcat[l] = (float*)take((size_t)(h->R + h->S) * 4);
    ok = G.wcat[l] && G.bcat[l];
  }
  if (!ok || !G.z || !G.skipsum || !G.logits || !G.sampled || !G.t_dev) { set_err("generation workspace allocation failed"); G.B = G.cap = 0; return WN_ERR_CUDA; }
  return WN_OK;
}

static void gen_dense(cudaStream_t st, const GenVec& v, int B, const int* t_dev) {
  const size_t smem = (size_t)GEN_ROWS * v.K * v.Cin * 4;
  static unsigned long long attr_devs = 0ull;
  if (tc_first_use_on_device(&attr_devs)) { cudaFuncSetAttribute(gen_dense_kernel, cudaFuncAttributeMaxDynamicSharedMemorySize, 160 * 1024); }
  gen_dense_kernel<<<dim3(cdiv(v.N, 32), cdiv(B, GEN_ROWS)), 256, smem, st>>>(v, B, t_dev);
}

static int gen_step(wn_handle* h, cudaStream_t st, int B, bool has_cb, bool sample, int deterministic, uint64_t seed, float* pred, long long pred_bstride,
                    int t0, bool write_audio) {
  wn_handle::Gen& G = h->gen;
  const int cap = G.cap, R = h->R, D = h->D;
  const int* t = G.t_dev;
  if (h->cfg.use_skip) gen_zero_kernel<<<cdiv(B * h->Sp, 256), 256, 0, st>>>(G.skipsum, B * h->Sp);
  gen_input_conv_kernel<<<cdiv(B * R, 128), 128, 0, st>>>(G.audio, cap, P_(h, h->input_conv.w_idx), P_(h, h->input_conv.b_idx), G.hist[0][0], R, h->K, B, t);
  for (int l = 0; l < h->L; ++l) {
    const BlockP& b = h->blocks[l];
    const int depth = (int)b.stack.size();
    for (int j = 0; j < depth; ++j) {
      const ConvP& c = b.stack[j];
      GenVec v{};
      v.in = G.hist[l][j]; v.in_bstride = (long long)cap * c.cin; v.in_tstride = c.cin; v.Cin = c.cin; v.K = c.K; v.dil = c.dil;
      v.W = P_(h, c.w_idx); v.bias = P_(h, c.b_idx); v.N = c.cout;
      if (j < depth - 1) {
        v.act = h->cfg.activation;
        v.out = G.hist[l][j + 1]; v.out_bstride = (long long)cap * D; v.out_tstride = D;
      } else {
        v.act = ACT_LINEAR;
        if (has_cb) { v.cbias = h->cb + (size_t)l * h->maxB * 2 * D; v.ldcb = 2 * D; }
        v.out = G.z; v.out_bstride = 2 * D; v.out_tstride = 0;
      }
      gen_dense(st, v, B, t);
    }
    {
      GenVec v{};
      v.in = G.z; v.in_bstride = 2 * D; v.in_tstride = 0; v.Cin = D; v.K = 1; v.dil = 1; v.in_gate = 1;
      v.act = ACT_LINEAR;
      v.out = G.hist[l + 1][0]; v.out_bstride = (long long)cap * R; v.out_tstride = R;
      if (h->cfg.use_residual) { v.res = G.hist[l][0]; v.res_bstride = (long long)cap * R; v.res_tstride = R; v.res_cols = R; }
      if (G.wcat[l]) {
        v.W = G.wcat[l]; v.bias = G.bcat[l]; v.N = R + h->S;
        v.acc = G.skipsum; v.acc_ld = h->Sp; v.acc_col0 = R;
      } else {
        v.W = P_(h, b.conv1.w_idx); v.bias = P_(h, b.conv1.b_idx); v.N = R;
        if (h->cfg.use_skip && h->alias_skip) { v.acc = G.skipsum; v.acc_ld = h->Sp; v.acc_col0 = -1; }
      }
      gen_dense(st, v, B, t);
    }
  }
  const float* hin = h->cfg.use_skip ? G.skipsum : G.hist[h->L][0];
  long long hin_b = h->cfg.use_skip ? h->Sp : (long long)cap * R;
  int hin_t = h->cfg.use_skip ? 0 : R;
  for (size_t i = 0; i < h->head.size(); ++i) {
    const ConvP& hc = h->head[i];
    const bool last = i + 1 == h->head.size();
    GenVec v{};
    v.in = hin; v.in_bstride = hin_b; v.in_tstride = hin_t; v.Cin = hc.cin; v.K = 1; v.dil = 1;
    v.W = P_(h, hc.w_idx); v.bias = P_(h, hc.b_idx); v.N = hc.cout; v.act = last ? ACT_LINEAR : h->cfg.activation;
    v.out = last ? G.logits : G.hbuf[i]; v.out_bstride = hc.cout; v.out_tstride = 0;
    gen_dense(st, v, B, t);
    hin = v.out; hin_b = hc.cout; hin_t = 0;
  }
  const wn_config& c = h->cfg;
  if (pred) gen_pred_kernel<<<B, 256, 0, st>>>(G.logits, h->Cout, c.sampling_function == WN_CATEGORICAL ? 1 : 0, pred, pred_bstride, t0, t);
  if (sample) {
    const int kind = c.sampling_function == WN_CATEGORICAL ? 0 : (c.sampling_function == WN_GAUSSIAN ? 2 : 1);
    sample_kernel<<<cdiv(B, 8), 256, 0, st>>>(G.logits, h->Cout, h->Cout, c.num_mixtures, kind, 1, c.bits, deterministic, seed, nullptr, 1, B, G.sampled, nullptr, t);
  }
  gen_advance_kernel<<<1, 64, 0, st>>>(G.audio, cap, G.sampled, B, write_audio ? 1 : 0, G.t_dev);
  CK(cudaGetLastError());
  return WN_OK;
}

extern "C" int wn_generate(wn_handle* h, const float* prime_dev, int n_prime, const float* cond_dev, int B, int length, int deterministic, uint64_t seed,
                           float* out_dev, float* pred_dev, const float* teacher_dev, void* stream) {
  if (!h) { set_err("null handle"); return WN_ERR_VALUE; }
  if (!h->cfg.has_head || !h->cfg.has_input_conv) { set_err("wn_generate needs a full model handle"); return WN_ERR_STATE; }
  if (h->cfg.conditioning && !cond_dev) { set_err("Conditioning must be provided."); return WN_ERR_VALUE; }
  if (!prime_dev || n_prime < 1 || B < 1 || B > 64 || B > h->maxB || length < 1 || (!out_dev && !pred_dev)) { set_err("bad generate arguments (1 <= batch <= min(64, max_batch))"); return WN_ERR_VALUE; }
  if ((size_t)GEN_ROWS * h->K * (h->R > h->D ? h->R : h->D) * 4 > 160 * 1024) { set_err("generation: K * channels too large for the step kernel"); return WN_ERR_UNSUPPORTED; }
  CK(cudaSetDevice(h->cfg.device));
  cudaStream_t user = (cudaStream_t)stream, st = h->own_stream;
  const int cap = n_prime + length + 1;
  RET(gen_alloc(h, B, cap));
  wn_handle::Gen& G = h->gen;
  CK(cudaEventRecord(h->ev_in, user)); CK(cudaStreamWaitEvent(st, h->ev_in, 0));
  for (size_t i = 0; i < G.allocs.size(); ++i) {  }
  CK(cudaMemsetAsync(G.audio, 0, (size_t)G.B * G.cap * 4, st));
  for (auto& hl : G.hist) for (float* p : hl) if (p) CK(cudaMemsetAsync(p, 0, (size_t)G.B * G.cap * 4 * ((p == hl[0]) ? h->R : h->D), st));
  CK(cudaMemsetAsync(G.t_dev, 0, 4, st));
  CK(cudaMemcpy2DAsync(G.audio, (size_t)G.cap * 4, prime_dev, (size_t)n_prime * 4, (size_t)n_prime * 4, B, cudaMemcpyDeviceToDevice, st));
  if (teacher_dev) CK(cudaMemcpy2DAsync(G.audio + n_prime, (size_t)G.cap * 4, teacher_dev, (size_t)length * 4, (size_t)length * 4, B, cudaMemcpyDeviceToDevice, st));
  bool has_cb = false;
  if (h->cfg.conditioning) {
    const float* cond = nullptr;
    RET(cond_forward(h, st, cond_dev, B, true, &cond));
    const int n = 2 * h->D;
    cond_bias_all<<<dim3(cdiv(B * n, 128), h->L), 128, 0, st>>>(cond, h->Cc, h->d_params, h->d_cond_offsets, h->cb, (long long)h->maxB * n, B, n);
    has_cb = true;
  }
// ... 791 lines not shown
```

Baseline: 11.18 million.

## Restructure stacked backward kernel to software-pipeline gate dgrad with previous tile's output GEMM

Rewrites the persistent stacked backward kernel so each role walks tiles in a skewed order: the gate dgrad of tile i is issued before the output GEMM of tile i-1. The unshifted dz operand now comes from global memory via TMA instead of the shared-memory dz slab handoff, and the V2 variant is removed. Output slots grow from 2 to 6 with deeper bulk-store pipelining, stages become 4, one warp is dropped, and band sizing changes. The intent is to hide the dz round-trip and the epilogue latency behind independent MMA work, at the cost of extra global and L2 traffic for dz.

Result: no change. 11.48 million, median of 6 (+2.6%).

```diff
diff --git a/wavenets_b200/csrc/gemm_tc_stack_bwd.cuh b/wavenets_b200/csrc/gemm_tc_stack_bwd.cuh
--- a/wavenets_b200/csrc/gemm_tc_stack_bwd.cuh
+++ b/wavenets_b200/csrc/gemm_tc_stack_bwd.cuh
@@ -11,6 +11,7 @@
 
 struct alignas(128) TcStackBwdLayer {
   CUtensorMap tmDX, tmDS, tmWdg, tmZf, tmZs, tmDZ, tmWb, tmDXp, tmO;
+  CUtensorMap tmDZf, tmDZs;
   int shift[TC_MAX_TAPS];
   int has_dx, has_ds, has_res;
   int wait_dx;
@@ -25,39 +26,35 @@
   int kb_dx, kb_ds;
   unsigned long long pol_dx, pol_ds, pol_w, pol_z, pol_dz_ld, pol_dz_st, pol_o;
   float drop_scale;
-  int relaxed_handoff;
   int band, nbands;
 };
 
-template <int D_, int R_, bool V2 = false> struct TcStackBwdCfg {
+template <int D_, int R_> struct TcStackBwdCfg {
   static constexpr int BM = 128, BK = 64;
   static constexpr int A_BYTES = BM * BK * 2;
   static constexpr int B_BYTES = 128 * BK * 2;
   static constexpr int STAGE_BYTES = A_BYTES + B_BYTES;
-  static constexpr int STAGES = V2 ? 5 : 3;
+  static constexpr int STAGES = 4;
   static constexpr int NSLAB = 2 * D_ / 64;
-  static constexpr int NPAIR = D_ / 64;
-  static constexpr int DZ_SLOTS = V2 ? 0 : 4;
-  static constexpr int DZ_BYTES = DZ_SLOTS * A_BYTES;
   static constexpr int PANEL = 128 * 64;
-  static constexpr int IN_SLOTS = 3, OUT_SLOTS = 2;
+  static constexpr int IN_SLOTS = 3, OUT_SLOTS = 6;
   static constexpr int TMEM_COLS = 512;
-  static constexpr int SMEM_BYTES = STAGES * STAGE_BYTES + DZ_BYTES + IN_SLOTS * 2 * PANEL + OUT_SLOTS * PANEL + 512;
+  static constexpr int SMEM_BYTES = STAGES * STAGE_BYTES + IN_SLOTS * 2 * PANEL + OUT_SLOTS * PANEL + 512;
+  static_assert(3 + OUT_SLOTS <= 16, "one named barrier per output panel slot, ids 3 ..");
   static_assert(D_ % 128 == 0 && D_ <= 256 && R_ % 64 == 0 && R_ <= 256, "stack backward kernel: D in {128,256}, R <= 256");
   static_assert(SMEM_BYTES <= 232448, "stack backward kernel does not fit shared memory");
 };
 
-template <int D_, int R_, bool V2>
-__global__ void __launch_bounds__(416, 1)
+template <int D_, int R_>
+__global__ void __launch_bounds__(384, 1)
 tc_stack_bwd_kernel(const TcStackBwdLayer* __restrict__ layers, int* __restrict__ flags_dx, int* __restrict__ flags_dz, const TcStackBwdParams p) {
-  using Cfg = TcStackBwdCfg<D_, R_, V2>;
-  constexpr int STAGES = Cfg::STAGES, NEPI = 8, NPAIR = Cfg::NPAIR;
+  using Cfg = TcStackBwdCfg<D_, R_>;
+  constexpr int STAGES = Cfg::STAGES, NEPI = 8;
   constexpr int KB_Z = Cfg::NSLAB;
   extern __shared__ __align__(1024) uint8_t smem_sb[];
   uint8_t* smem = smem_sb;
   if ((smem_u32(smem) & 1023u) != 0u) { if (threadIdx.x == 0) printf("libwavenet_b200: dynamic shared memory is not 1024-byte aligned\n"); __trap(); }
-  uint8_t* dzbuf = smem + STAGES * Cfg::STAGE_BYTES;
-  uint8_t* in_ring = dzbuf + Cfg::DZ_BYTES;
+  uint8_t* in_ring = smem + STAGES * Cfg::STAGE_BYTES;
   uint8_t* out_ring = in_ring + Cfg::IN_SLOTS * 2 * Cfg::PANEL;
   uint64_t* full_bar = (uint64_t*)(out_ring + Cfg::OUT_SLOTS * Cfg::PANEL);
   uint64_t* empty_bar = full_bar + STAGES;
@@ -68,19 +65,7 @@
   uint64_t* in_full = out_empty + 1;
   uint64_t* in_empty = in_full + Cfg::IN_SLOTS;
   uint64_t* oslot_empty = in_empty + Cfg::IN_SLOTS;
-  uint64_t* slab_done = oslot_empty + Cfg::OUT_SLOTS;
-  uint64_t* slab_full = slab_done + 2;
-  uint64_t* slab_cons = slab_full + 2;
-  uint64_t* slab_free = slab_cons + 2;
-  uint64_t* a_done = slab_free + 2;
-  uint64_t* a_ready = a_done + STAGES;
-  uint64_t* sfree = a_ready + STAGES;
-  uint32_t* tmem_ptr = (uint32_t*)(sfree + STAGES);
-  auto tile_ksteps = [&](const TcStackBwdLayer& Ly, int& n_dg, int& n_un, int& n_sh) {
-    if (Ly.kind) { n_dg = 0; n_un = 0; n_sh = p.nseg * Ly.kb_tap; }
-    else { n_dg = (Ly.has_dx ? p.kb_dx : 0) + (Ly.has_ds ? p.kb_ds : 0); n_un = KB_Z; n_sh = (p.nseg - 1) * KB_Z; }
-  };
-  auto ring_adv = [&](int& rs, uint32_t& rp, int n) { rs += n; while (rs >= STAGES) { rs -= STAGES; rp ^= 1u; } };
+  uint32_t* tmem_ptr = (uint32_t*)(oslot_empty + Cfg::OUT_SLOTS);
 
   const int warp = threadIdx.x >> 5, lane = threadIdx.x & 31;
   const uint32_t crank = cluster_ctarank();
@@ -106,14 +91,18 @@
     tb = p.tiles_t - 1 - (mr - b * p.tiles_t);
     mt = b * p.tiles_t + tb;
   };
+  auto walk = [&](auto&& dg, auto&& out) {
+    for (int i = 0; i <= n_tiles; ++i) {
+      if (i < n_tiles) { int ly, mt, b, tb; locate(i, ly, mt, b, tb); if (!layers[ly].kind) dg(i, ly, mt, b, tb); }
+      if (i > 0) { int ly, mt, b, tb; locate(i - 1, ly, mt, b, tb); out(i - 1, ly, mt, b, tb); }
+    }
+  };
 
   if (warp == 1 && lane == 0) {
     for (int i = 0; i < STAGES; ++i) { mbar_init(&full_bar[i], 1); mbar_init(&empty_bar[i], 1); }
     mbar_init(dg_full, 1); mbar_init(dg_empty, NEPI * 2); mbar_init(out_full, 1); mbar_init(out_empty, NEPI * 2);
     for (int i = 0; i < Cfg::IN_SLOTS; ++i) { mbar_init(&in_full[i], 1); mbar_init(&in_empty[i], NEPI); }
     for (int i = 0; i < Cfg::OUT_SLOTS; ++i) mbar_init(&oslot_empty[i], 1);
-    for (int i = 0; i < 2; ++i) { mbar_init(&slab_done[i], NEPI); mbar_init(&slab_full[i], 2); mbar_init(&slab_cons[i], 1); mbar_init(&slab_free[i], 1); }
-    for (int i = 0; i < STAGES; ++i) { mbar_init(&a_done[i], NEPI); mbar_init(&a_ready[i], 2); mbar_init(&sfree[i], 1); }
     mbar_fence_init();
   }
   if (warp == 2) tmem_alloc_pair<Cfg::TMEM_COLS>(tmem_ptr);
@@ -137,40 +126,11 @@
     if (lane == 0) {
       int stage = 0; uint32_t phase = 0;
       auto next = [&]() { if (++stage == STAGES) { stage = 0; phase ^= 1; } };
-      uint32_t un_pend = 0u, un_wpar = 0u, un_npar = 0u;
-      auto stage_wait = [&]() {
-        mbar_wait(&empty_bar[stage], phase ^ 1);
-        if (V2 && ((un_pend >> stage) & 1u)) { mbar_wait(&sfree[stage], (un_wpar >> stage) & 1u); un_pend &= ~(1u << stage); }
-      };
       SBT_DECL(4)
       constexpr int WDG_BYTES = (D_ / 2) * 64 * 2, WB_BYTES = (R_ / 2) * 64 * 2;
-      for (int j = 0; j < n_tiles; ++j) {
-        int ly, mt, b, tb;
-        locate(j, ly, mt, b, tb);
+      auto dg = [&](int, int ly, int mt, int b, int tb) {
         const TcStackBwdLayer& Ly = layers[ly];
         const int t0 = tb * (2 * Cfg::BM) + pair_row0;
-        if (Ly.kind) {
-          for (int s = 0; s < p.nseg; ++s) {
-            const int lo = tb * (2 * Cfg::BM) + Ly.shift[s];
-            const int t_lo = lo / (2 * Cfg::BM);
-            int t_hi = (lo + 2 * Cfg::BM - 1) / (2 * Cfg::BM);
-            if (t_hi > p.tiles_t - 1) t_hi = p.tiles_t - 1;
-            SBT(0)
-            for (int tt = t_lo; tt <= t_hi; ++tt) wait_flag(flags_dx + (size_t)(ly + 1) * p.num_mtiles + b * p.tiles_t + tt, ly + 1, b * p.tiles_t + tt);
-            SBT(1)
-          }
-          fence_proxy_async_global();
-          for (int s = 0; s < p.nseg; ++s)
-            for (int kb = 0; kb < Ly.kb_tap; ++kb) {
-              stage_wait();
-              uint8_t* sa = smem + stage * Cfg::STAGE_BYTES;
-              if (leader) mbar_expect_tx(&full_bar[stage], 2 * (Cfg::A_BYTES + WB_BYTES));
-              tma_load_3d_pair_h(sa, &Ly.tmDZ, &full_bar[stage], kb * 64, t0 + Ly.shift[s], b, p.pol_dz_ld);
-              tma_load_2d_pair_h(sa + Cfg::A_BYTES, &Ly.tmWb, &full_bar[stage], (s * Ly.kb_tap + kb) * 64, (int)crank * (R_ / 2), p.pol_w);
-              next();
-            }
-          continue;
-        }
         if (Ly.has_dx) {
           if (Ly.wait_dx) {
             SBT(0)
@@ -179,7 +139,7 @@
             SBT(1)
           }
           for (int kb = 0; kb < p.kb_dx; ++kb) {
-            stage_wait();
+            mbar_wait(&empty_bar[stage], phase ^ 1);
             uint8_t* sa = smem + stage * Cfg::STAGE_BYTES;
             if (leader) mbar_expect_tx(&full_bar[stage], 2 * (Cfg::A_BYTES + WDG_BYTES));
             tma_load_4d_pair_h(sa, &Ly.tmDX, &full_bar[stage], kb * 64, t0, b, 0, p.pol_dx);
@@ -190,7 +150,7 @@
         if (Ly.has_ds) {
           const int k0 = (Ly.has_dx && !Ly.alias) ? p.kb_dx * 64 : 0;
           for (int kb = 0; kb < p.kb_ds; ++kb) {
-            stage_wait();
+            mbar_wait(&empty_bar[stage], phase ^ 1);
             uint8_t* sa = smem + stage * Cfg::STAGE_BYTES;
             if (leader) mbar_expect_tx(&full_bar[stage], 2 * (Cfg::A_BYTES + WDG_BYTES));
             tma_load_4d_pair_h(sa, &Ly.tmDS, &full_bar[stage], kb * 64, t0, b, 0, p.pol_ds);
@@ -198,40 +158,35 @@
             next();
           }
         }
-        const int kloc = (p.nseg - 1) * 2 * D_;
-        for (int pr = 0; pr < NPAIR; ++pr) {
-          for (int hh = 0; hh < 2; ++hh) {
-            const int slab = hh == 0 ? pr : NPAIR + pr;
-            stage_wait();
-            uint8_t* sa = smem + stage * Cfg::STAGE_BYTES;
-            if (leader) mbar_expect_tx(&full_bar[stage], 2 * WB_BYTES);
-            tma_load_2d_pair_h(sa + Cfg::A_BYTES, &Ly.tmWb, &full_bar[stage], kloc + slab * 64, (int)crank * (R_ / 2), p.pol_w);
-            if (V2) {
-              un_wpar = (un_wpar & ~(1u << stage)) | (((un_npar >> stage) & 1u) << stage);
-              un_npar ^= 1u << stage; un_pend |= 1u << stage;
-            }
-            next();
-          }
-        }
-        for (int s = 0; s < p.nseg - 1; ++s) {
+      };
+      auto out = [&](int, int ly, int, int b, int tb) {
+        const TcStackBwdLayer& Ly = layers[ly];
+        const int t0 = tb * (2 * Cfg::BM) + pair_row0;
+        const int kb_tap = Ly.kind ? Ly.kb_tap : KB_Z;
+        const int fl = Ly.kind ? ly + 1 : ly;
+        const int* fbase = (Ly.kind ? flags_dx : flags_dz) + (size_t)fl * p.num_mtiles + b * p.tiles_t;
+        for (int i = 0; i < p.nseg; ++i) {
+          const int s = Ly.kind ? i : (i == 0 ? p.nseg - 1 : i - 1);
           const int lo = tb * (2 * Cfg::BM) + Ly.shift[s];
           const int t_lo = lo / (2 * Cfg::BM);
           int t_hi = (lo + 2 * Cfg::BM - 1) / (2 * Cfg::BM);
           if (t_hi > p.tiles_t - 1) t_hi = p.tiles_t - 1;
           SBT(0)
-          for (int tt = t_lo; tt <= t_hi; ++tt) wait_flag(flags_dz + (size_t)ly * p.num_mtiles + b * p.tiles_t + tt, ly, b * p.tiles_t + tt);
+          for (int tt = t_lo; tt <= t_hi; ++tt) wait_flag(fbase + tt, fl, b * p.tiles_t + tt);
           fence_proxy_async_global();
-          SBT(2)
-          for (int kb = 0; kb < KB_Z; ++kb) {
-            stage_wait();
+          SBT(Ly.kind ? 1 : 2)
+          for (int kb = 0; kb < kb_tap; ++kb) {
+            const int col = (!Ly.kind && s == p.nseg - 1) ? (kb & 1) * D_ + (kb >> 1) * 64 : kb * 64;
+            mbar_wait(&empty_bar[stage], phase ^ 1);
             uint8_t* sa = smem + stage * Cfg::STAGE_BYTES;
             if (leader) mbar_expect_tx(&full_bar[stage], 2 * (Cfg::A_BYTES + WB_BYTES));
-            tma_load_3d_pair_h(sa, &Ly.tmDZ, &full_bar[stage], kb * 64, t0 + Ly.shift[s], b, p.pol_dz_ld);
-            tma_load_2d_pair_h(sa + Cfg::A_BYTES, &Ly.tmWb, &full_bar[stage], s * 2 * D_ + kb * 64, (int)crank * (R_ / 2), p.pol_w);
+            tma_load_3d_pair_h(sa, &Ly.tmDZ, &full_bar[stage], col, t0 + Ly.shift[s], b, p.pol_dz_ld);
+            tma_load_2d_pair_h(sa + Cfg::A_BYTES, &Ly.tmWb, &full_bar[stage], s * kb_tap * 64 + col, (int)crank * (R_ / 2), p.pol_w);
             next();
           }
         }
-      }
+      };
+      walk(dg, out);
       SBT(0)
 #ifdef TC_TIMELINE
       if (blockIdx.x == 0 || blockIdx.x == 41)
@@ -244,11 +199,9 @@
       constexpr uint32_t idesc_o = umma_idesc_bf16(256, R_, 0, 0);
       const uint32_t t_dg = tmem_base, t_out = tmem_base + 256u;
       int stage = 0; uint32_t phase = 0;
-      uint32_t n_sf[2] = {0u, 0u};
       uint32_t ng = 0u;
-      uint32_t ar_par = 0u;
       SBT_DECL(10)
-      auto kstep = [&](uint32_t d_tmem, uint32_t idesc, bool a_from_dz, int slot, bool first, uint64_t* extra0, uint64_t* extra1) {
+      auto kstep = [&](uint32_t d_tmem, uint32_t idesc, bool first, uint64_t* extra) {
 #ifdef TC_TIMELINE
         const long long w0 = clock64();
 #endif
@@ -259,150 +212,110 @@
         tc_fence_after();
         if (elect_one()) {
           const uint32_t sa = smem_u32(smem + stage * Cfg::STAGE_BYTES);
-          const uint32_t a_addr = a_from_dz ? smem_u32(dzbuf) + (uint32_t)slot * (uint32_t)Cfg::A_BYTES : sa;
-          const uint64_t adesc = umma_smem_desc(a_addr, 16, 1024);
+          const uint64_t adesc = umma_smem_desc(sa, 16, 1024);
           const uint64_t bdesc = umma_smem_desc(sa + Cfg::A_BYTES, 16, 1024);
 #pragma unroll
           for (int k = 0; k < Cfg::BK / 16; ++k)
             umma_bf16_pair(d_tmem, adesc + (uint64_t)(2 * k), bdesc + (uint64_t)(2 * k), idesc, (first && k == 0) ? 0u : 1u);
           umma_commit_pair(&empty_bar[stage]);
-          if (extra0) umma_commit_pair(extra0);
-          if (extra1) umma_commit_pair(extra1);
+          if (extra) umma_commit_pair(extra);
         }
         __syncwarp();
         if (++stage == STAGES) { stage = 0; phase ^= 1; }
       };
-      for (int j = 0; j < n_tiles; ++j) {
-        int ly, mt, b, tb;
-        locate(j, ly, mt, b, tb);
+      auto dg = [&](int, int ly, int, int, int) {
         const TcStackBwdLayer& Ly = layers[ly];
-        const uint32_t par = (uint32_t)(j & 1);
-        if (Ly.kind) {
-          SBT(2)
-          mbar_wait(out_empty, par ^ 1);
-          SBT(3)
-          tc_fence_after();
-          const int ks_p = p.nseg * Ly.kb_tap;
-          for (int ks = 0; ks < ks_p; ++ks) kstep(t_out, idesc_o, false, 0, ks == 0, ks == ks_p - 1 ? out_full : nullptr, nullptr);
-          SBT(7)
-          continue;
-        }
         const uint32_t gpar = ng & 1u; ++ng;
         SBT(0)
         mbar_wait(dg_empty, gpar ^ 1);
         SBT(1)
         tc_fence_after();
         const int ks_dg = (Ly.has_dx ? p.kb_dx : 0) + (Ly.has_ds ? p.kb_ds : 0);
-        for (int ks = 0; ks < ks_dg; ++ks) kstep(t_dg, idesc_g, false, 0, ks == 0, ks == ks_dg - 1 ? dg_full : nullptr, nullptr);
+        for (int ks = 0; ks < ks_dg; ++ks) kstep(t_dg, idesc_g, ks == 0, ks == ks_dg - 1 ? dg_full : nullptr);
         SBT(2)
-        mbar_wait(out_empty, par ^ 1);
+      };
+      auto out = [&](int j, int ly, int, int, int) {
+        const TcStackBwdLayer& Ly = layers[ly];
+        SBT(0)
+        mbar_wait(out_empty, (uint32_t)(j & 1) ^ 1u);
         SBT(3)
         tc_fence_after();
-        const int ks_sh = (p.nseg - 1) * KB_Z;
-        bool first = true;
-        if constexpr (V2) {
-          for (int q = 0; q < KB_Z; ++q) {
-            if ((q & 1) == 0) { mbar_wait(&a_ready[stage], (ar_par >> stage) & 1u); ar_par ^= 1u << stage; }
-            SBT(5)
-            tc_fence_after();
-            const bool last = ks_sh == 0 && q == KB_Z - 1;
-            kstep(t_out, idesc_o, false, 0, first, last ? out_full : nullptr, nullptr); first = false;
-            SBT(6)
-          }
-        } else
-        for (int pr = 0; pr < NPAIR; ++pr) {
-          const int ps = pr & 1;
-          mbar_wait(&slab_full[ps], n_sf[ps] & 1u); ++n_sf[ps];
-          SBT(5)
-          tc_fence_after();
-          const bool last = ks_sh == 0 && pr == NPAIR - 1;
-          kstep(t_out, idesc_o, true, 2 * ps, first, nullptr, nullptr); first = false;
-          kstep(t_out, idesc_o, true, 2 * ps + 1, false, &slab_cons[ps], last ? out_full : nullptr);
-          SBT(6)
-        }
-        for (int ks = 0; ks < ks_sh; ++ks) kstep(t_out, idesc_o, false, 0, false, ks == ks_sh - 1 ? out_full : nullptr, nullptr);
+        const int n_un = Ly.kind ? 0 : KB_Z;
+        const int n = p.nseg * (Ly.kind ? Ly.kb_tap : KB_Z);
+        for (int ks = 0; ks < n; ++ks) {
+          kstep(t_out, idesc_o, ks == 0, ks == n - 1 ? out_full : nullptr);
+          if (ks == n_un - 1) { SBT(6) }
+        }
         SBT(7)
-      }
+      };
+      walk(dg, out);
 #ifdef TC_TIMELINE
       if (lane == 0 && (blockIdx.x == 0 || blockIdx.x == 40))
-        printf("SBWD cta %d mma: tiles %d  wait_dg_empty %lld  DG ksteps %lld  wait_out_empty %lld  wait_slab_full %lld  unshifted %lld  shifted %lld  (of the ksteps: wait_full_bar %lld)\n",
-               blockIdx.x, n_tiles, sbt[1], sbt[2], sbt[3], sbt[5], sbt[6], sbt[7], sbt[9]);
+        printf("SBWD cta %d mma: tiles %d  wait_dg_empty %lld  DG ksteps %lld  wait_out_empty %lld  unshifted %lld  shifted %lld  (of the ksteps: wait_full_bar %lld)\n",
+               blockIdx.x, n_tiles, sbt[1], sbt[2], sbt[3], sbt[6], sbt[7], sbt[9]);
 #endif
     }
   } else if (warp == 2) {
     int oslot = 0;
-    uint64_t* pend = nullptr;
-    uint64_t* pend2 = nullptr;
-    auto committed = [&](uint64_t* rel, uint64_t* rel2 = nullptr) {
+    auto put = [&]() { const int s = oslot; if (++oslot == Cfg::OUT_SLOTS) oslot = 0; return s; };
+    uint64_t* pend[3][2];
+    int npend = 0;
+    auto release_oldest = [&]() {
+      mbar_arrive(pend[0][0]); if (pend[0][1]) mbar_arrive(pend[0][1]);
+      for (int i = 1; i < npend; ++i) { pend[i - 1][0] = pend[i][0]; pend[i - 1][1] = pend[i][1]; }
+      --npend;
+    };
+    auto committed = [&](uint64_t* r0, uint64_t* r1) {
       bulk_commit_group();
-      if (pend) { bulk_wait_group_read<1>(); mbar_arrive(pend); if (pend2) mbar_arrive(pend2); }
-      pend = rel; pend2 = rel2;
-    };
-    int s_rs = 0; uint32_t s_rp = 0u;
+      pend[npend][0] = r0; pend[npend][1] = r1; ++npend;
+      if (npend == 3) { bulk_wait_group_read<2>(); release_oldest(); }
+    };
     auto publish = [&](int* flag) {
       bulk_wait_group<0>();
-      if (pend) { mbar_arrive(pend); if (pend2) mbar_arrive(pend2); pend = nullptr; pend2 = nullptr; }
+      while (npend > 0) release_oldest();
       fence_proxy_async_global();
       __threadfence();
       red_release_gpu_add(flag, 1);
     };
-    for (int j = 0; j < n_tiles; ++j) {
-      int ly, mt, b, tb;
-      locate(j, ly, mt, b, tb);
+    auto dg = [&](int, int ly, int mt, int b, int tb) {
       const TcStackBwdLayer& Ly = layers[ly];
       const int t0 = tb * (2 * Cfg::BM) + pair_row0;
-      int n_dg, n_un, n_sh;
-      tile_ksteps(Ly, n_dg, n_un, n_sh);
-      if (!Ly.kind) {
-      int u_rs = s_rs; uint32_t u_rp = s_rp;
-      ring_adv(u_rs, u_rp, n_dg);
-      for (int pr = 0; pr < NPAIR; ++pr) {
-        const int ps = pr & 1;
-        if constexpr (V2) {
-          named_bar_sync(8 + pr, NEPI * 32 + 32);
-          const int sf = u_rs; ring_adv(u_rs, u_rp, 1);
-          const int ss = u_rs; ring_adv(u_rs, u_rp, 1);
-          if (lane == 0) {
-            tma_store_3d_h(smem + sf * Cfg::STAGE_BYTES, &Ly.tmDZ, pr * 64, t0, b, p.pol_dz_st);
-            tma_store_3d_h(smem + ss * Cfg::STAGE_BYTES, &Ly.tmDZ, D_ + pr * 64, t0, b, p.pol_dz_st);
-            committed(&sfree[sf], &sfree[ss]);
-          }
-        } else {
-        named_bar_sync(8 + ps, NEPI * 32 + 32);
+      for (int step = 0; step < D_ / 32; ++step) {
+        const int sf = put(), sg = put();
+        named_bar_sync(3 + sf, NEPI * 32 + 32);
         if (lane == 0) {
-          tma_store_3d_h(dzbuf + (2 * ps) * Cfg::A_BYTES, &Ly.tmDZ, pr * 64, t0, b, p.pol_dz_st);
-          tma_store_3d_h(dzbuf + (2 * ps + 1) * Cfg::A_BYTES, &Ly.tmDZ, D_ + pr * 64, t0, b, p.pol_dz_st);
-          committed(&slab_free[ps]);
-        }
+          tma_store_3d_h(out_ring + sf * Cfg::PANEL, &Ly.tmDZf, step * 32, t0, b, p.pol_dz_st);
+          tma_store_3d_h(out_ring + sg * Cfg::PANEL, &Ly.tmDZs, step * 32, t0, b, p.pol_dz_st);
+          committed(&oslot_empty[sf], &oslot_empty[sg]);
         }
         __syncwarp();
       }
       if (lane == 0) publish(flags_dz + (size_t)ly * p.num_mtiles + mt);
       __syncwarp();
-      }
+    };
+    auto out = [&](int, int ly, int mt, int b, int tb) {
+      const TcStackBwdLayer& Ly = layers[ly];
+      const int t0 = tb * (2 * Cfg::BM) + pair_row0;
       for (int step = 0; step < R_ / 32; ++step) {
-        named_bar_sync(3 + oslot, NEPI * 32 + 32);
+        const int so = put();
+        named_bar_sync(3 + so, NEPI * 32 + 32);
         if (lane == 0) {
-          tma_store_3d_h(out_ring + oslot * Cfg::PANEL, &Ly.tmO, step * 32, t0, b, p.pol_o);
-          committed(&oslot_empty[oslot]);
+          tma_store_3d_h(out_ring + so * Cfg::PANEL, &Ly.tmO, step * 32, t0, b, p.pol_o);
+          committed(&oslot_empty[so], nullptr);
         }
         __syncwarp();
-        if (++oslot == Cfg::OUT_SLOTS) oslot = 0;
       }
       if (lane == 0) publish(flags_dx + (size_t)ly * p.num_mtiles + mt);
       __syncwarp();
-      ring_adv(s_rs, s_rp, n_dg + n_un + n_sh);
-    }
+    };
+    walk(dg, out);
     if (lane == 0) bulk_wait_group<0>();
   } else if (warp == 3) {
     if (lane == 0) {
       int islot = 0; uint32_t iphase = 0;
-      for (int j = 0; j < n_tiles; ++j) {
-        int ly, mt, b, tb;
-        locate(j, ly, mt, b, tb);
+      auto dg = [&](int, int ly, int, int b, int tb) {
         const TcStackBwdLayer& Ly = layers[ly];
         const int t0 = tb * (2 * Cfg::BM) + pair_row0;
-        if (!Ly.kind)
         for (int step = 0; step < D_ / 32; ++step) {
           mbar_wait(&in_empty[islot], iphase ^ 1);
           mbar_expect_tx(&in_full[islot], 2u * Cfg::PANEL);
@@ -411,49 +324,23 @@
           tma_load_3d_h(dst + Cfg::PANEL, &Ly.tmZs, &in_full[islot], step * 32, t0, b, p.pol_z);
           if (++islot == Cfg::IN_SLOTS) { islot = 0; iphase ^= 1; }
         }
-        if (Ly.out_mode) {
-          if (Ly.in_flag_layer >= 0) {
-            wait_flag(flags_dx + (size_t)Ly.in_flag_layer * p.num_mtiles + mt, Ly.in_flag_layer, mt);
-            fence_proxy_async_global();
-          }
-          for (int step = 0; step < R_ / 32; ++step) {
-            mbar_wait(&in_empty[islot], iphase ^ 1);
-            mbar_expect_tx(&in_full[islot], (uint32_t)Cfg::PANEL);
-            tma_load_3d_h(in_ring + islot * 2 * Cfg::PANEL, &Ly.tmDXp, &in_full[islot], step * 32, t0, b, p.pol_dx);
-            if (++islot == Cfg::IN_SLOTS) { islot = 0; iphase ^= 1; }
-          }
-        }
-      }
-    }
-  } else if (warp == 12) {
-    if (lane == 0) {
-      uint32_t n_sd[2] = {0u, 0u};
-      int h_rs = 0; uint32_t h_rp = 0u, ad_par = 0u;
-      for (int j = 0; j < n_tiles; ++j) {
-        int n_dg, n_un, n_sh;
-        { int ly, mt, b, tb; locate(j, ly, mt, b, tb); tile_ksteps(layers[ly], n_dg, n_un, n_sh); }
-        if constexpr (V2) {
-          int u_rs = h_rs; uint32_t u_rp = h_rp;
-          ring_adv(u_rs, u_rp, n_dg);
-          for (int q = 0; q < n_un; q += 2) {
-            mbar_wait(&a_done[u_rs], (ad_par >> u_rs) & 1u); ad_par ^= 1u << u_rs;
-            if (leader) mbar_arrive(&a_ready[u_rs]);
-            else if (p.relaxed_handoff) mbar_arrive_remote_relaxed(&a_ready[u_rs], 0u);
-            else mbar_arrive_remote(&a_ready[u_rs], 0u);
-            ring_adv(u_rs, u_rp, 2);
-          }
-          ring_adv(h_rs, h_rp, n_dg + n_un + n_sh);
-          continue;
-        }
-        if (n_un == 0) continue;
-        for (int pr = 0; pr < NPAIR; ++pr) {
-          const int ps = pr & 1;
-          mbar_wait(&slab_done[ps], n_sd[ps] & 1u); ++n_sd[ps];
-          if (leader) mbar_arrive(&slab_full[ps]);
-          else if (p.relaxed_handoff) mbar_arrive_remote_relaxed(&slab_full[ps], 0u);
-          else mbar_arrive_remote(&slab_full[ps], 0u);
-        }
-      }
+      };
+      auto out = [&](int, int ly, int mt, int b, int tb) {
+        const TcStackBwdLayer& Ly = layers[ly];
+        if (!Ly.out_mode) return;
+        const int t0 = tb * (2 * Cfg::BM) + pair_row0;
+        if (Ly.in_flag_layer >= 0) {
+          wait_flag(flags_dx + (size_t)Ly.in_flag_layer * p.num_mtiles + mt, Ly.in_flag_layer, mt);
+          fence_proxy_async_global();
+        }
+        for (int step = 0; step < R_ / 32; ++step) {
+          mbar_wait(&in_empty[islot], iphase ^ 1);
+          mbar_expect_tx(&in_full[islot], (uint32_t)Cfg::PANEL);
+          tma_load_3d_h(in_ring + islot * 2 * Cfg::PANEL, &Ly.tmDXp, &in_full[islot], step * 32, t0, b, p.pol_dx);
+          if (++islot == Cfg::IN_SLOTS) { islot = 0; iphase ^= 1; }
+        }
+      };
+      walk(dg, out);
     }
   } else if (warp >= 4 && warp < 12) {
     const int e = warp - 4;
@@ -464,179 +351,131 @@
     const uint32_t sw = (uint32_t)((row >> 1) & 3);
     const uint32_t u0 = (uint32_t)(2 * q), u1 = u0 + 1;
     const uint32_t off0 = row_off + ((u0 ^ sw) << 4), off1 = row_off + ((u1 ^ sw) << 4);
-    const uint32_t grow = (uint32_t)row * 128u, gsw = (uint32_t)(row & 7);
     int islot = 0; uint32_t iphase = 0;
     int oslot = 0; uint32_t ophase = 0;
-    uint32_t n_use[2] = {0u, 0u};
     uint32_t nge = 0u;
-    int e_rs = 0; uint32_t e_rp = 0u;
-    uint32_t eu_pend = 0u, eu_wpar = 0u, eu_npar = 0u;
-    uint8_t* slab_dst[2] = {nullptr, nullptr};
-    int slab_st[2] = {0, 0};
+    auto take = [&]() {
+      const int s = oslot;
+      mbar_wait(&oslot_empty[s], ophase ^ 1);
+      if (++oslot == Cfg::OUT_SLOTS) { oslot = 0; ophase ^= 1; }
+      return s;
+    };
+    auto pack16 = [&](int slot, const float* v) {
+      uint8_t* ob = out_ring + slot * Cfg::PANEL;
+      uint4 a, c;
+      a.x = pack_bf16x2(v[0], v[1]); a.y = pack_bf16x2(v[2], v[3]); a.z = pack_bf16x2(v[4], v[5]); a.w = pack_bf16x2(v[6], v[7]);
+      c.x = pack_bf16x2(v[8], v[9]); c.y = pack_bf16x2(v[10], v[11]); c.z = pack_bf16x2(v[12], v[13]); c.w = pack_bf16x2(v[14], v[15]);
+      *reinterpret_cast<uint4*>(ob + off0) = a;
+      *reinterpret_cast<uint4*>(ob + off1) = c;
+    };
     const TcEpiGateBwd<true>::Params pg{D_};
     const uint32_t lane_base = (uint32_t)(quarter * 32) << 16;
     SBT_DECL(10)
-    for (int j = 0; j < n_tiles; ++j) {
-      const uint32_t par = (uint32_t)(j & 1);
-      int out_mode, out_act, kind;
-      int n_dg, n_un, n_sh;
-      const uint8_t* mrow = nullptr;
-      {
-        int ly, mt, b, tb;
-        locate(j, ly, mt, b, tb);
-        out_mode = layers[ly].out_mode; out_act = layers[ly].act; kind = layers[ly].kind;
-        tile_ksteps(layers[ly], n_dg, n_un, n_sh);
-        const int tt = tb * (2 * Cfg::BM) + pair_row0 + row;
-        if (layers[ly].mask && tt < p.T && b < p.B) mrow = layers[ly].mask + ((size_t)b * p.T + tt) * R_;
-      }
-      if (!kind) {
+    auto dg = [&](int, int, int, int, int) {
       const uint32_t gpar = nge & 1u; ++nge;
       SBT(0)
       mbar_wait(dg_full, gpar);
       SBT(1)
       tc_fence_after();
-      int u_rs = e_rs; uint32_t u_rp = e_rp;
-      ring_adv(u_rs, u_rp, n_dg);
+      TmemAccRow acc{tmem_base + lane_base, true};
+#pragma unroll 1
+      for (int step = 0; step < D_ / 32; ++step) {
+        float in[2][16];
+        float out[2][16];
+        SBT(2)
+        mbar_wait(&in_full[islot], iphase);
+        SBT(3)
+        {
+          const uint8_t* ib = in_ring + islot * 2 * Cfg::PANEL;
+#pragma unroll
+          for (int k = 0; k < 2; ++k) {
+            const uint4 a = *reinterpret_cast<const uint4*>(ib + k * Cfg::PANEL + off0);
+            const uint4 c = *reinterpret_cast<const uint4*>(ib + k * Cfg::PANEL + off1);
+            const uint32_t w[8] = {a.x, a.y, a.z, a.w, c.x, c.y, c.z, c.w};
+#pragma unroll
+            for (int i = 0; i < 8; ++i) {
+              in[k][2 * i] = __uint_as_float(w[i] << 16);
+              in[k][2 * i + 1] = __uint_as_float(w[i] & 0xffff0000u);
+            }
+          }
+        }
+        __syncwarp();
+        if (lane == 0) mbar_arrive(&in_empty[islot]);
+        if (++islot == Cfg::IN_SLOTS) { islot = 0; iphase ^= 1; }
+        TcEpiGateBwd<true>::chunk(pg, acc, 0, step * 32 + q * 16, 0, 0, 3u, in, out, nullptr);
+        SBT(2)
+        const int sf = take(), sg = take();
+        SBT(4)
+        pack16(sf, out[0]);
+        pack16(sg, out[1]);
+        fence_proxy_async();
+        named_bar_arrive(3 + sf, NEPI * 32 + 32);
+      }
+      tc_fence_before();
+      __syncwarp();
+      if (lane == 0) mbar_arrive_remote_relaxed(dg_empty, 0u);
+    };
+    auto out = [&](int j, int ly, int, int b, int tb) {
+      const TcStackBwdLayer& Ly = layers[ly];
+      const int out_mode = Ly.out_mode, out_act = Ly.act;
+      const uint8_t* mrow = nullptr;
       {
-        TmemAccRow acc{tmem_base + lane_base, true};
+        const int tt = tb * (2 * Cfg::BM) + pair_row0 + row;
+        if (Ly.mask && tt < p.T && b < p.B) mrow = Ly.mask + ((size_t)b * p.T + tt) * R_;
+      }
+      SBT(0)
+      mbar_wait(out_full, (uint32_t)(j & 1));
+      SBT(5)
+      tc_fence_after();
+      TmemAccRow acc{tmem_base + 256u + lane_base, true};
 #pragma unroll 1
-        for (int step = 0; step < D_ / 32; ++step) {
-          const int pr = step >> 1, ps = pr & 1;
-          float in[2][16];
-          float out[2][16];
-          SBT(2)
+      for (int step = 0; step < R_ / 32; ++step) {
+        float v[16];
+        acc.load16(step * 32 + q * 16, v);
+        if (mrow) {
+          const uint4 mk = __ldg(reinterpret_cast<const uint4*>(mrow + step * 32 + q * 16));
+          const uint32_t mw[4] = {mk.x, mk.y, mk.z, mk.w};
+#pragma unroll
+          for (int i = 0; i < 16; ++i) v[i] = ((mw[i >> 2] >> (8 * (i & 3))) & 0xffu) ? v[i] * p.drop_scale : 0.f;
+        }
+        if (out_mode) {
           mbar_wait(&in_full[islot], iphase);
-          SBT(3)
-          {
-            const uint8_t* ib = in_ring + islot * 2 * Cfg::PANEL;
+          const uint8_t* ib = in_ring + islot * 2 * Cfg::PANEL;
+          const uint4 a = *reinterpret_cast<const uint4*>(ib + off0);
+          const uint4 c = *reinterpret_cast<const uint4*>(ib + off1);
+          const uint32_t w[8] = {a.x, a.y, a.z, a.w, c.x, c.y, c.z, c.w};
+          float y[16];
 #pragma unroll
-            for (int k = 0; k < 2; ++k) {
-              const uint4 a = *reinterpret_cast<const uint4*>(ib + k * Cfg::PANEL + off0);
-              const uint4 c = *reinterpret_cast<const uint4*>(ib + k * Cfg::PANEL + off1);
-              const uint32_t w[8] = {a.x, a.y, a.z, a.w, c.x, c.y, c.z, c.w};
+          for (int i = 0; i < 8; ++i) {
+            y[2 * i] = __uint_as_float(w[i] << 16);
+            y[2 * i + 1] = __uint_as_float(w[i] & 0xffff0000u);
+          }
+          if (out_mode == 1) {
 #pragma unroll
-              for (int i = 0; i < 8; ++i) {
-                in[k][2 * i] = __uint_as_float(w[i] << 16);
-                in[k][2 * i + 1] = __uint_as_float(w[i] & 0xffff0000u);
-              }
-            }
+            for (int i = 0; i < 16; ++i) v[i] += y[i];
+          } else {
+            wn_act_grad16(out_act, y, v);
           }
           __syncwarp();
           if (lane == 0) mbar_arrive(&in_empty[islot]);
           if (++islot == Cfg::IN_SLOTS) { islot = 0; iphase ^= 1; }
-          TcEpiGateBwd<true>::chunk(pg, acc, 0, step * 32 + q * 16, 0, 0, 3u, in, out, nullptr);
-          SBT(2)
-          if constexpr (V2) {
-            if ((step & 1) == 0) {
-#pragma unroll
-              for (int k = 0; k < 2; ++k) {
-                mbar_wait(&empty_bar[u_rs], u_rp ^ 1u);
-                if ((eu_pend >> u_rs) & 1u) { mbar_wait(&sfree[u_rs], (eu_wpar >> u_rs) & 1u); eu_pend &= ~(1u << u_rs); }
-                eu_wpar = (eu_wpar & ~(1u << u_rs)) | (((eu_npar >> u_rs) & 1u) << u_rs);
-                eu_npar ^= 1u << u_rs; eu_pend |= 1u << u_rs;
-                slab_st[k] = u_rs; slab_dst[k] = smem + u_rs * Cfg::STAGE_BYTES;
-                ring_adv(u_rs, u_rp, 1);
-              }
-            }
-          } else
-          if ((step & 1) == 0 && n_use[ps] > 0) {
-            mbar_wait(&slab_cons[ps], (n_use[ps] - 1u) & 1u);
-            mbar_wait(&slab_free[ps], (n_use[ps] - 1u) & 1u);
-          }
-          SBT(4)
-          {
-            const int ch = (step & 1) * 32 + q * 16;
-            const uint32_t j0 = (uint32_t)(ch >> 3);
-#pragma unroll
-            for (int k = 0; k < 2; ++k) {
-              uint8_t* gs = (V2 ? slab_dst[k] : dzbuf + (2 * ps + k) * Cfg::A_BYTES) + grow;
-              uint4 a, c;
-              a.x = pack_bf16x2(out[k][0], out[k][1]); a.y = pack_bf16x2(out[k][2], out[k][3]);
-              a.z = pack_bf16x2(out[k][4], out[k][5]); a.w = pack_bf16x2(out[k][6], out[k][7]);
-              c.x = pack_bf16x2(out[k][8], out[k][9]); c.y = pack_bf16x2(out[k][10], out[k][11]);
-              c.z = pack_bf16x2(out[k][12], out[k][13]); c.w = pack_bf16x2(out[k][14], out[k][15]);
-              *reinterpret_cast<uint4*>(gs + ((j0 ^ gsw) << 4)) = a;
-              *reinterpret_cast<uint4*>(gs + (((j0 + 1) ^ gsw) << 4)) = c;
-            }
-          }
-          if (step & 1) {
-            fence_proxy_async();
-            named_bar_arrive(8 + (V2 ? pr : ps), NEPI * 32 + 32);
-            __syncwarp();
-            if constexpr (V2) {
-              if (lane == 0) mbar_arrive(&a_done[slab_st[0]]);
-            } else {
-              if (lane == 0) mbar_arrive(&slab_done[ps]);
-            }
-            ++n_use[ps];
-          }
-        }
-      }
-      tc_fence_before();
-      __syncwarp();
-      if (lane == 0) mbar_arrive_remote_relaxed(dg_empty, 0u);
-      }
-      SBT(2)
-      mbar_wait(out_full, par);
-      SBT(5)
-      tc_fence_after();
-      {
-        TmemAccRow acc{tmem_base + 256u + lane_base, true};
-#pragma unroll 1
-        for (int step = 0; step < R_ / 32; ++step) {
-          float v[16];
-          acc.load16(step * 32 + q * 16, v);
-          if (mrow) {
-            const uint4 mk = __ldg(reinterpret_cast<const uint4*>(mrow + step * 32 + q * 16));
-            const uint32_t mw[4] = {mk.x, mk.y, mk.z, mk.w};
-#pragma unroll
-            for (int i = 0; i < 16; ++i) v[i] = ((mw[i >> 2] >> (8 * (i & 3))) & 0xffu) ? v[i] * p.drop_scale : 0.f;
-          }
-          if (out_mode) {
-            mbar_wait(&in_full[islot], iphase);
-            const uint8_t* ib = in_ring + islot * 2 * Cfg::PANEL;
-            const uint4 a = *reinterpret_cast<const uint4*>(ib + off0);
-            const uint4 c = *reinterpret_cast<const uint4*>(ib + off1);
-            const uint32_t w[8] = {a.x, a.y, a.z, a.w, c.x, c.y, c.z, c.w};
-            float y[16];
-#pragma unroll
-            for (int i = 0; i < 8; ++i) {
-              y[2 * i] = __uint_as_float(w[i] << 16);
-              y[2 * i + 1] = __uint_as_float(w[i] & 0xffff0000u);
-            }
-            if (out_mode == 1) {
-#pragma unroll
-              for (int i = 0; i < 16; ++i) v[i] += y[i];
-            } else {
-              wn_act_grad16(out_act, y, v);
-            }
-            __syncwarp();
-            if (lane == 0) mbar_arrive(&in_empty[islot]);
-            if (++islot == Cfg::IN_SLOTS) { islot = 0; iphase ^= 1; }
-          }
-          uint8_t* ob = out_ring + oslot * Cfg::PANEL;
-          SBT(6)
-          mbar_wait(&oslot_empty[oslot], ophase ^ 1);
-          SBT(7)
-          uint4 a, c;
-          a.x = pack_bf16x2(v[0], v[1]); a.y = pack_bf16x2(v[2], v[3]); a.z = pack_bf16x2(v[4], v[5]); a.w = pack_bf16x2(v[6], v[7]);
-          c.x = pack_bf16x2(v[8], v[9]); c.y = pack_bf16x2(v[10], v[11]); c.z = pack_bf16x2(v[12], v[13]); c.w = pack_bf16x2(v[14], v[15]);
-          *reinterpret_cast<uint4*>(ob + off0) = a;
-          *reinterpret_cast<uint4*>(ob + off1) = c;
-          fence_proxy_async();
-          named_bar_arrive(3 + oslot, NEPI * 32 + 32);
-          if (++oslot == Cfg::OUT_SLOTS) { oslot = 0; ophase ^= 1; }
-        }
+        }
+        SBT(6)
+        const int so = take();
+        SBT(7)
+        pack16(so, v);
+        fence_proxy_async();
+        named_bar_arrive(3 + so, NEPI * 32 + 32);
       }
       tc_fence_before();
       __syncwarp();
       if (lane == 0) mbar_arrive_remote_relaxed(out_empty, 0u);
-      ring_adv(e_rs, e_rp, n_dg + n_un + n_sh);
       SBT(6)
-    }
+    };
+    walk(dg, out);
 #ifdef TC_TIMELINE
     if (lane == 0 && warp == 4 && (blockIdx.x == 0 || blockIdx.x == 41))
-      printf("SBWD cta %d epilogue warp 4: wait_dg_full %lld  DG epi work %lld (+ wait z panels %lld, wait slab slot %lld)  wait_out_full %lld  OUT epi work %lld (+ wait out slot %lld)\n",
+      printf("SBWD cta %d epilogue warp 4: wait_dg_full %lld  DG epi work %lld (+ wait z panels %lld, wait panel slots %lld)  wait_out_full %lld  OUT epi work %lld (+ wait out slot %lld)\n",
              blockIdx.x, sbt[1], sbt[2], sbt[3], sbt[4], sbt[5], sbt[6], sbt[7]);
 #endif
   }
@@ -695,18 +534,21 @@
       const CUtensorMap* mG = tc_slab_map(tc, d.gin, d.D, d.D, d.T, d.B);
       if (!mG) return -10;
       t.tmDZ = *mG; t.kb_tap = d.D / 64;
-      t.tmDX = *mG; t.tmDS = *mG; t.tmWdg = *mWb; t.tmZf = *mO; t.tmZs = *mO;
+      t.tmDX = *mG; t.tmDS = *mG; t.tmWdg = *mWb; t.tmZf = *mO; t.tmZs = *mO; t.tmDZf = *mO; t.tmDZs = *mO;
       continue;
     }
     const CUtensorMap* mDZ = tc_slab_map(tc, d.dz, 2 * d.D, 2 * d.D, d.T, d.B);
     const TcEpiIo zf{d.z, 2 * d.D, d.D, 0}, zs{d.z + d.D, 2 * d.D, d.D, 0};
     const CUtensorMap* mZf = tc_panel_map(tc, zf, d.T, d.B);
     const CUtensorMap* mZs = tc_panel_map(tc, zs, d.T, d.B);
+    const TcEpiIo dzf{d.dz, 2 * d.D, d.D, 0}, dzs{d.dz + d.D, 2 * d.D, d.D, 0};
+    const CUtensorMap* mDZf = tc_panel_map(tc, dzf, d.T, d.B);
+    const CUtensorMap* mDZs = tc_panel_map(tc, dzs, d.T, d.B);
     uint64_t wd[2] = {(uint64_t)d.k_dg, (uint64_t)d.D}, ws[1] = {(uint64_t)d.k_dg * 2};
     uint32_t wb[2] = {64, (uint32_t)(D_ / 2)};
     const CUtensorMap* mWdg = tc.get(d.Wdg, 2, wd, ws, wb);
-    if (!mDZ || !mZf || !mZs || !mWdg) return -10;
-    t.tmDZ = *mDZ; t.tmZf = *mZf; t.tmZs = *mZs; t.tmWdg = *mWdg;
+    if (!mDZ || !mZf || !mZs || !mDZf || !mDZs || !mWdg) return -10;
+    t.tmDZ = *mDZ; t.tmZf = *mZf; t.tmZs = *mZs; t.tmDZf = *mDZf; t.tmDZs = *mDZs; t.tmWdg = *mWdg;
     t.tmDX = *mDZ; t.tmDS = *mDZ;
     if (d.dxo) {
       const CUtensorMap* m = tc_act_map(tc, d.dxo, d.R, d.R, d.T, d.B, 1, 0, 128);
@@ -735,15 +577,15 @@
   return 0;
 }
 
-template <int D_, int R_, bool V2>
+template <int D_, int R_>
 static int tc_stack_bwd_launch_t(cudaStream_t st, const TcStackBwdPlan& plan, const TcStackBwdDesc& d0) {
-  using Cfg = TcStackBwdCfg<D_, R_, V2>;
+  using Cfg = TcStackBwdCfg<D_, R_>;
   TcStackBwdParams p{};
   p.B = d0.B; p.T = d0.T; p.tiles_t = (d0.T + 255) / 256; p.num_mtiles = d0.B * p.tiles_t; p.L = plan.L;
   p.nseg = d0.nseg; p.kb_dx = d0.R / 64; p.kb_ds = d0.S / 64; p.drop_scale = d0.drop_scale;
   p.pol_dx = tc_policy(TC_L2_NORMAL); p.pol_ds = tc_policy(TC_L2_LAST); p.pol_w = tc_policy(TC_L2_LAST); p.pol_z = tc_policy(TC_L2_FIRST);
   p.pol_dz_ld = tc_policy(TC_L2_NORMAL); p.pol_dz_st = tc_policy(TC_L2_LAST); p.pol_o = tc_policy(TC_L2_LAST);
-  auto kern = tc_stack_bwd_kernel<D_, R_, V2>;
+  auto kern = tc_stack_bwd_kernel<D_, R_>;
   static unsigned long long attr_devs = 0ull;
   if (tc_first_use_on_device(&attr_devs)) {
     cudaError_t e = cudaFuncSetAttribute(kern, cudaFuncAttributeMaxDynamicSharedMemorySize, Cfg::SMEM_BYTES);
@@ -752,16 +594,13 @@
   const int pairs = tc_num_sms() / 2;
   if (p.num_mtiles <= pairs) return -100;
   {
-    static int relaxed = -1;
-    if (relaxed < 0) { const char* e = getenv("WN_TC_HANDOFF_RELAXED"); relaxed = (e && e[0] == '1') ? 1 : 0; }
-    p.relaxed_handoff = relaxed;
     static int band_target = -1;
     if (band_target < 0) { const char* e = getenv("WN_TC_SB_BAND"); band_target = e ? atoi(e) : 128; }
     int nb = band_target > 0 ? p.num_mtiles / band_target : 1;
     if (nb < 1) nb = 1;
     for (; nb > 1; --nb) {
       const int bw = (p.num_mtiles + nb - 1) / nb;
-      if (bw > pairs && p.num_mtiles - (nb - 1) * bw > pairs) break;
+      if (bw >= 3 * pairs && p.num_mtiles - (nb - 1) * bw >= 3 * pairs) break;
     }
     p.nbands = nb; p.band = (p.num_mtiles + nb - 1) / nb;
   }
@@ -771,7 +610,7 @@
     int& max_clusters = max_clusters_dev[tc_current_device()];
     if (tc_first_use_on_device(&mc_devs)) {
       cudaLaunchConfig_t oc{};
-      oc.gridDim = dim3(tc_num_sms()); oc.blockDim = dim3(416); oc.dynamicSmemBytes = Cfg::SMEM_BYTES;
+      oc.gridDim = dim3(tc_num_sms()); oc.blockDim = dim3(384); oc.dynamicSmemBytes = Cfg::SMEM_BYTES;
       cudaLaunchAttribute oa[1];
       oa[0].id = cudaLaunchAttributeClusterDimension;
       oa[0].val.clusterDim.x = 2; oa[0].val.clusterDim.y = 1; oa[0].val.clusterDim.z = 1;
@@ -785,7 +624,7 @@
   const size_t nflags = (size_t)plan.L * plan.num_mtiles;
   if (cudaMemsetAsync(plan.d_flags, 0, 2 * nflags * sizeof(int), st) != cudaSuccess) return -14;
   cudaLaunchConfig_t cfg{};
-  cfg.gridDim = dim3(2 * pairs); cfg.blockDim = dim3(416); cfg.dynamicSmemBytes = Cfg::SMEM_BYTES; cfg.stream = st;
+  cfg.gridDim = dim3(2 * pairs); cfg.blockDim = dim3(384); cfg.dynamicSmemBytes = Cfg::SMEM_BYTES; cfg.stream = st;
   cudaLaunchAttribute attr[2];
   cfg.attrs = attr; cfg.numAttrs = tc_launch_attrs(attr, 2);
   cudaError_t e = cudaLaunchKernelEx(&cfg, kern, (const TcStackBwdLayer*)plan.d_layers, plan.d_flags, plan.d_flags + nflags, p);
@@ -799,8 +638,8 @@
   if (d.D == 128 && d.R == 128) return tc_stack_bwd_build_t<128, 128>(tc, descs, plan);
   return -100;
 }
-static inline int tc_stack_bwd_launch(cudaStream_t st, const TcStackBwdPlan& plan, const TcStackBwdDesc& d, bool v2) {
-  if (d.D == 256 && d.R == 256) return v2 ? tc_stack_bwd_launch_t<256, 256, true>(st, plan, d) : tc_stack_bwd_launch_t<256, 256, false>(st, plan, d);
-  if (d.D == 128 && d.R == 128) return v2 ? tc_stack_bwd_launch_t<128, 128, true>(st, plan, d) : tc_stack_bwd_launch_t<128, 128, false>(st, plan, d);
+static inline int tc_stack_bwd_launch(cudaStream_t st, const TcStackBwdPlan& plan, const TcStackBwdDesc& d) {
+  if (d.D == 256 && d.R == 256) return tc_stack_bwd_launch_t<256, 256>(st, plan, d);
+  if (d.D == 128 && d.R == 128) return tc_stack_bwd_launch_t<128, 128>(st, plan, d);
   return -100;
 }
diff --git a/wavenets_b200/csrc/wn_api.cu b/wavenets_b200/csrc/wn_api.cu
--- a/wavenets_b200/csrc/wn_api.cu
+++ b/wavenets_b200/csrc/wn_api.cu
@@ -198,7 +198,7 @@
   int stack_fwd_layers = 0;
   int use_stack_fwd = 1;
   std::vector<TcStackPlan> stack_plans;
-  int use_stack_bwd = 2, stack_bwd_layers = 0;
+  int use_stack_bwd = 1, stack_bwd_layers = 0;
   std::vector<TcStackBwdPlan> stack_bwd_plans;
   int tile_gate_bwd = 0, tile_dgrad = 0;
   int fused_fwd_launches = 0;
@@ -1893,7 +1893,7 @@
         if (sp) {
           struct Label { wn_handle* h; Label(wn_handle* h_) : h(h_) { h->cur_label = "stack_bwd"; } ~Label() { h->cur_label = "misc"; } } lab(h);
           LaunchScope ls(h, st, CLS_DILATED);
-          r = tc_stack_bwd_launch(st, *sp, bdescs[0], h->use_stack_bwd >= 2);
+          r = tc_stack_bwd_launch(st, *sp, bdescs[0]);
           if (r == 0) { stacked = true; h->stack_bwd_layers = h->L; }
           else if (r == -100) h->launches--;
           else { set_err("stack backward launch failed (%d): %s", r, tc_last_error()); return WN_ERR_CUDA; }
```
